# ilirlikalla/Smith-Waterman-FPGA-module

Hardware: AMD Instinct MI355X
Metric: GCUPS (higher is better)
Workload: dtype f16

## Files before the change

smith-waterman-fpga-module_amd/csrc/swbank_bank.h:

```cpp
#ifndef SWBANK_BANK_H
#define SWBANK_BANK_H

#include <dlfcn.h>
#include <hip/hip_runtime.h>
#include <rccl/rccl.h>

#include <algorithm>
#include <cmath>
#include <cstdarg>
#include <cstdio>
#include <cstdlib>
#include <cstring>
#include <atomic>
#include <condition_variable>
#include <functional>
#include <memory>
#include <mutex>
#include <numeric>
#include <thread>
#include <chrono>
#include <vector>
#if defined(__SSE2__)
#include <emmintrin.h>
#endif
#if defined(__x86_64__)
#include <immintrin.h>
#endif

#include "swbank.h"
#include "swbank_align.h"
#include "swbank_internal.h"
#include "swbank_pack.h"

extern "C" int swk_has_variant(int R, int RB, int col0, int prof, int gotoh, int f16);
extern "C" hipError_t swk_launch_wave(int K, int col0, int prof, int gotoh, int f16,
                                      const void* edge_in, void* edge_out, uint32_t ecols,
                                      int accum, const uint8_t* res,
                                      const uint64_t* offs, const uint32_t* lens, size_t n,
                                      const uint32_t* qtab, uint32_t nv, uint32_t S, uint32_t O,
                                      uint32_t E, uint32_t PS, uint32_t pad, int32_t* scores,
                                      int packed, const uint32_t* fb_qtab, uint32_t fb_nv,
                                      uint32_t fb_PS, int32_t fb_thresh,
                                      const SwkWaveSplit* split, uint32_t ulen,
                                      uint32_t ustride, int half, hipStream_t st);
extern "C" hipError_t swk_launch_score(int R, int RB, int col0, int prof, int gotoh, int f16,
                                       const uint8_t* res, const uint64_t* offs,
                                       const uint32_t* lens, size_t n, const uint32_t* qtab,
                                       uint32_t nv, uint32_t S, uint32_t O, uint32_t E,
                                       uint32_t PS, uint32_t pad, int W, int32_t* scores,
                                       const void* edge_in, void* edge_out, uint32_t ecols,
                                       int accum, int packed, const uint32_t* idx,
                                       const uint32_t* nidx, uint32_t idx_base,
                                       const uint32_t* ident, int pair, uint32_t pS1,
                                       uint32_t pS2, uint32_t ulen, uint32_t ustride, uint32_t nq,
                                       uint32_t qwords, size_t sstride, hipStream_t st);
extern "C" unsigned swk_bal_slots(int W, uint32_t PS, int trim);
extern "C" unsigned swk_wave_half_grid(int gotoh, uint32_t prof_bytes, int W);
extern "C" hipError_t swk_bal_plan_uniform(void* plan, uint32_t ntiles, uint32_t K, uint32_t G,
                                           hipStream_t st);
extern "C" hipError_t swk_launch_pair_bal(const uint8_t* res, const uint64_t* offs,
                                          const uint32_t* lens, size_t n, const uint32_t* qtab,
                                          uint32_t nv, uint32_t S, uint32_t O, uint32_t E,
                                          uint32_t PS, uint32_t pad, int W, int32_t* scores,
                                          uint32_t pS1, uint32_t pS2, uint32_t ulen,
                                          uint32_t ustride, uint32_t* flag, uint32_t* state,
                                          uint32_t gen, unsigned grid, const uint32_t* idx,
                                          const uint32_t* nidx, const uint32_t* ident,
                                          const void* plan, uint32_t* fault, uint32_t poll_limit,
                                          uint32_t stall, int trim, uint32_t packed,
                                          const uint32_t* sidx, hipStream_t st);
extern "C" hipError_t swk_best_hit(const int32_t* scores, const uint64_t* ids, size_t n,
                                   unsigned long long* key, uint64_t* out, uint64_t* out_index,
                                   hipStream_t st);
extern "C" hipError_t swk_best_part(const int32_t* scores, size_t n, size_t base,
                                    unsigned long long* key, hipStream_t st);
extern "C" hipError_t swk_best_finalize(const unsigned long long* key, const uint64_t* ids,
                                        uint64_t* out, uint64_t* out_index, hipStream_t st);
extern "C" hipError_t swk_sort_lens(const uint32_t* lens, size_t n, uint32_t max_len,
                                    uint32_t* perm, uint32_t* perm_n, uint32_t* ident,
                                    uint32_t* scratch, hipStream_t st, void* plan = nullptr,
                                    unsigned G = 0);
extern "C" size_t swk_sort_scratch_bytes(void);
extern "C" hipError_t swk_flag_high(const int32_t* scores, size_t n, int32_t thresh,
                                    uint32_t* idx, uint32_t* count, hipStream_t st);
extern "C" size_t swk_i32_waves(size_t n, uint32_t scols, size_t budget_bytes);
extern "C" hipError_t swk_launch_i32(int gotoh, const uint8_t* res, const uint64_t* offs,
                                     const uint32_t* lens, size_t n, int packed,
                                     const uint32_t* idx, const uint32_t* nidx, uint32_t idx_base,
                                     const void* prof, uint32_t nstrips, uint32_t qlen,
                                     uint32_t pad, uint32_t O, uint32_t E, int32_t* scores,
                                     void* scratch, uint32_t scols, size_t waves, hipStream_t st);

extern "C" size_t swk_top_state_words(void);
extern "C" hipError_t swk_top_hits(const int32_t* scores, const uint64_t* ids, size_t n, size_t nq,
                                   size_t k, int32_t min_score, unsigned long long* state,
                                   unsigned long long* keys, uint64_t* hits, int32_t* hit_scores,
                                   uint64_t* hit_ids, uint32_t* counts, hipStream_t st);

inline int env_int(const char* name, int dflt) {
  const char* v = std::getenv(name);
  return (v && *v) ? std::atoi(v) : dflt;
}

struct PhaseTrace {
  const char* path = std::getenv("SWBANK_TRACE_FILE");
  std::chrono::steady_clock::time_point t0 = std::chrono::steady_clock::now();
  std::vector<std::pair<const char*, double>> marks;
  std::mutex mu;
  void mark(const char* what) { mark_at(what, std::chrono::steady_clock::now()); }
  void mark_at(const char* what, std::chrono::steady_clock::time_point t) {
    if (!path) return;
    std::lock_guard<std::mutex> g(mu);
    marks.push_back({what, std::chrono::duration<double, std::micro>(t - t0).count()});
  }
  ~PhaseTrace() {
    if (!path || marks.empty()) return;
    if (FILE* f = std::fopen(path, "a")) {
      for (auto& m : marks) std::fprintf(f, "%s %.1f\n", m.first, m.second);
      std::fprintf(f, "--\n");
      std::fclose(f);
    }
  }
};
inline thread_local PhaseTrace* g_trace = nullptr;
inline void trace_mark(const char* what) {
  if (g_trace) g_trace->mark(what);
}

inline bool poison_buffers() {
  const char* v = std::getenv("SWBANK_POISON");
  return v && v[0] == '1';
}

template <typename T>
struct DevBuf {
  T* p = nullptr;
  size_t cap = 0;
  hipError_t reserve(size_t n) {
    if (n <= cap) return hipSuccess;
    if (p) (void)hipFree(p);
    p = nullptr;
    cap = 0;
    size_t want = std::max<size_t>(n, 64);
    hipError_t e = hipMalloc(reinterpret_cast<void**>(&p), want * sizeof(T));
    if (e == hipSuccess) cap = want;
    if (e == hipSuccess && poison_buffers()) {
      e = hipMemset(p, 0x3C, want * sizeof(T));
      if (e == hipSuccess) e = hipStreamSynchronize(nullptr);
    }
    return e;
  }
  void release() {
    if (p) (void)hipFree(p);
// ... 128 lines not shown
    }
    cv_.notify_one();
  }
  sw_status wait(size_t k) {
    while (done_.load(std::memory_order_acquire) < k) {
#if defined(__SSE2__)
      _mm_pause();
#endif
    }
    return st_.load(std::memory_order_acquire);
  }
  sw_status wait_all() { return wait(posted_); }
  void reset() {
    wait_all();
    posted_ = 0;
    done_.store(0);
    st_.store(SW_OK);
  }

 private:
  void loop(int device) {
    (void)hipSetDevice(device);
    for (;;) {
      std::function<sw_status()> f;
      {
        std::unique_lock<std::mutex> l(m_);
        cv_.wait(l, [&] { return stop_ || !q_.empty(); });
        if (q_.empty()) return;
        f = std::move(q_.front());
        q_.erase(q_.begin());
      }
      if (st_.load(std::memory_order_relaxed) == SW_OK) {
        const sw_status s = f();
        if (s != SW_OK) st_.store(s, std::memory_order_release);
      }
      done_.fetch_add(1, std::memory_order_acq_rel);
    }
  }
  std::mutex m_;
  std::condition_variable cv_;
  std::vector<std::function<sw_status()>> q_;
  bool stop_ = false;
  size_t posted_ = 0;
  std::atomic<size_t> done_{0};
  std::atomic<sw_status> st_{SW_OK};
  std::thread th_;
};

struct sw_bank {
  sw_config cfg{};
  int device = 0;
  int cus = 0;
  hipStream_t stream = nullptr;
  char err[512] = {0};

  bool have_pen = false;
  int alpha = SW_DNA_ALPHA;
  std::vector<int8_t> matrix;
  int32_t gap_open = 0, gap_extend = 0;

  bool have_query = false;
  uint64_t qid = 0;
  std::vector<uint8_t> query;
  std::vector<std::vector<uint8_t>> qset;
  bool mq_ready = false;
  DevBuf<uint32_t> mqtab, mqtab16;
  size_t mq_words = 0;
  DevBuf<uint32_t> mqpair;
  size_t mq_pair_words = 0;
  int mq_pair_segs = 0, mq_pair_rows = 0;
  uint32_t mq_pS1 = 0, mq_pS2 = 0;

  bool dirty = true;
  int R = 32, RB = 4, W = 1, col0 = 0, prof = 0;
  uint32_t S = 0, O = 0, E = 0, nv = 0, PS = 0, pad = 4;
  int32_t smax = 0;
  DevBuf<uint32_t> qtab;
  bool f16 = false;
  uint32_t nv16 = 0, PS16 = 0;
  int32_t f16_neg = 0;
  DevBuf<uint32_t> qtab16;
  DevBuf<uint32_t> qpair;
  uint32_t pair_bytes = 0, pS1 = 0, pS2 = 0;
  DevBuf<uint32_t> fb_idx, fb_cnt;
  bool i32_ready = false;
  uint32_t i32_strips = 0;
  DevBuf<uint2> i32prof, i32scr;
  DevBuf<unsigned long long> best_key;
  bool al_ready = false;
  DevBuf<uint8_t> al_tab, al_res;
  DevBuf<uint2> al_scr;
  DevBuf<uint32_t> al_dirs, al_lens, al_cig, al_list;
  DevBuf<uint64_t> al_offs;
  DevBuf<sw_alignment> al_out;
  DevBuf<SwkAlignPlan> al_plan;
  DevBuf<unsigned long long> top_state, top_keys;
  DevBuf<int32_t> top_scores, top_hsc;
  DevBuf<uint64_t> top_hits;
  DevBuf<uint32_t> top_cnt;
  hipEvent_t ev_top = nullptr;
  struct Seg { int W; size_t off, off16; };
  std::vector<Seg> segs;
  DevBuf<uint2> edge[2];
  int wK = 0;
  int wsegs = 1;
  size_t wseg_words = 0, wseg_words16 = 0;
  uint32_t wPS = 0;
  DevBuf<uint32_t> wtab;
  DevBuf<uint32_t> wtab16;
  uint32_t wPS16 = 0;
  int sK[3] = {0, 0, 0};
  size_t sseg_words[3] = {0, 0, 0}, sseg_words16[3] = {0, 0, 0};
  uint32_t sPS[3] = {0, 0, 0}, sPS16[3] = {0, 0, 0};
  DevBuf<uint32_t> stab[3], stab16[3];
  DevBuf<uint2> sring;
  DevBuf<uint32_t> tprog;

  static constexpr int NSLOT = 3, NDSLOT = 6;
  hipStream_t copy_stream = nullptr;
  hipEvent_t h2d_done[NSLOT] = {}, kern_done[NDSLOT] = {};
  PinBuf hslot[NSLOT], hscores;
  std::vector<std::vector<uint32_t>> mlist;
  std::vector<std::vector<uint8_t>> mstage;
  std::vector<std::vector<uint32_t>> mbad;
  std::vector<hipEvent_t> out_ev;
  hipStream_t out_stream = nullptr;
  hipStream_t stream2 = nullptr;
  hipEvent_t ev_s2 = nullptr;
  double host_pack_ms = 0;
  int feed_dslots = NSLOT;
  DevBuf<uint8_t> dslot[NDSLOT];
  DevBuf<uint32_t> sortscr[NDSLOT];
  DevBuf<uint8_t> sbuf;
  UcBuf sflag;
  DevBuf<SwkStreamChunk> sdrec;
  DevBuf<uint32_t> sctr;
  hipStream_t kstream = nullptr;
  PinBuf srec, shflag{hipHostMallocCoherent};
  PinBuf shscores{hipHostMallocCoherent};
  std::vector<hipEvent_t> sev;
  std::unique_ptr<HostPool> pool;
  std::unique_ptr<Launcher> launcher;

  DevBuf<uint8_t> res;
  DevBuf<uint64_t> offs;
  DevBuf<uint32_t> lens;
  DevBuf<int32_t> scores;
  DevBuf<uint8_t> gres;
  DevBuf<uint64_t> goffs;
  DevBuf<uint32_t> glens;

  char last_kernel[160] = {0};

  int best_kind = 0;
  uint64_t best_id = 0, best_index = 0;
  int32_t best_score = 0;
  DevBuf<uint64_t> best_dev;
  hipEvent_t best_ev = nullptr;

  std::vector<sw_bank*> kids;
  std::unique_ptr<HostPool> dpool;
  std::vector<void*> comms;
  bool rccl_gather = false;
  unsigned pool_threads = 0;
  DevBuf<int32_t> grecv;
  PinBuf hrecv;
// ... 178 lines not shown
```

smith-waterman-fpga-module_amd/csrc/swbank_bank.hip:

```cpp
#include "swbank_bank.h"

sw_status fail(sw_bank* b, sw_status st, const char* fmt, ...) {
  if (b) {
    va_list ap;
    va_start(ap, fmt);
    vsnprintf(b->err, sizeof(b->err), fmt, ap);
    va_end(ap);
  }
  return st;
}

extern "C" int32_t sw_device_count(void) {
  int n = 0;
  if (hipGetDeviceCount(&n) != hipSuccess) return 0;
  return n;
}

static sw_status check_device(int dev) {
  int ndev = 0;
  if (hipGetDeviceCount(&ndev) != hipSuccess || ndev <= 0) return SW_ERR_NO_DEVICE;
  if (dev < 0 || dev >= ndev) return SW_ERR_NO_DEVICE;
  hipDeviceProp_t prop;
  if (hipGetDeviceProperties(&prop, dev) != hipSuccess) return SW_ERR_NO_DEVICE;
  if (std::strncmp(prop.gcnArchName, "gfx950", 6) != 0) return SW_ERR_NO_DEVICE;
// ... 63 lines not shown
        sw_bank_destroy(b);
        return SW_ERR_UNSUPPORTED;
      }
      if (b->comms.empty())
        snprintf(b->err, sizeof(b->err), "RCCL unavailable (%s), gathering with device copies",
                 r.ok ? r.errorString(nr) : r.err);
    }
    (void)hipSetDevice(b->device);
    *out = b;
    return SW_OK;
  }

  int dev = cfg.device;
  if (dev < 0 && hipGetDevice(&dev) != hipSuccess) return SW_ERR_NO_DEVICE;
  const sw_status dst = check_device(dev);
  if (dst != SW_OK) return dst;

  sw_bank* b = new (std::nothrow) sw_bank();
  if (!b) return SW_ERR_NOMEM;
  b->cfg = cfg;
  b->device = dev;
  if (hipSetDevice(dev) != hipSuccess ||
      hipStreamCreateWithFlags(&b->stream, hipStreamNonBlocking) != hipSuccess ||
      hipStreamCreateWithFlags(&b->copy_stream, hipStreamNonBlocking) != hipSuccess ||
      hipStreamCreateWithFlags(&b->out_stream, hipStreamNonBlocking) != hipSuccess ||
      hipStreamCreateWithFlags(&b->stream2, hipStreamNonBlocking) != hipSuccess) {
    for (hipStream_t* x : {&b->stream, &b->copy_stream, &b->out_stream, &b->stream2})
      if (*x) (void)hipStreamDestroy(*x);
    delete b;
    return SW_ERR_HIP;
  }
  b->alpha = cfg.alphabet == SW_ALPHABET_DNA ? SW_DNA_ALPHA : SW_PROTEIN_ALPHA;
  if (hipDeviceGetAttribute(&b->cus, hipDeviceAttributeMultiprocessorCount, dev) != hipSuccess)
    b->cus = 0;
  if (cfg.alphabet == SW_ALPHABET_PROTEIN) {
    int8_t m[SW_PROTEIN_ALPHA * SW_PROTEIN_ALPHA];
    sw_fill_matrix(SW_ALPHABET_PROTEIN, 0, 0, m);
    b->matrix.assign(m, m + sizeof(m));
    b->gap_open = -11;
    b->gap_extend = -1;
    b->have_pen = true;
  }
  *out = b;
  return SW_OK;
}

extern "C" void sw_bank_destroy(sw_bank* b) {
  DevGuard dev_guard(b);
  if (!b) return;
  if (b->is_multi() || !b->comms.empty()) {
    const Rccl& r = rccl();
    for (void* c : b->comms) (void)r.commDestroy(static_cast<ncclComm_t>(c));
    (void)hipSetDevice(b->device);
    if (b->ev_used) (void)hipEventSynchronize(b->ev_used);
    if (b->ev_join) (void)hipEventDestroy(b->ev_join);
    if (b->ev_used) (void)hipEventDestroy(b->ev_used);
    for (sw_bank* k : b->kids) sw_bank_destroy(k);
    b->dpool.reset();
    b->pool.reset();
    (void)hipSetDevice(b->device);
    b->grecv.release();
    b->hrecv.release();
    b->res.release();
    b->offs.release();
    b->lens.release();
    b->dperm.release();
    b->dsort.release();
    delete b;
    return;
  }
  (void)hipSetDevice(b->device);
  if (b->stream) (void)hipStreamSynchronize(b->stream);
  if (b->ev_top) (void)hipEventSynchronize(b->ev_top);
  uint64_t nl;
  double pm, sm;
  (void)sw_bank_timing(b, &nl, &pm, &sm);
  b->faultw.release();
  b->qtab.release();
  b->qtab16.release();
  b->mqtab.release();
  b->mqtab16.release();
  b->mqpair.release();
  b->qpair.release();
  b->stage.release();
  if (b->ev_ready) (void)hipEventDestroy(b->ev_ready);
  if (b->ev_used) (void)hipEventDestroy(b->ev_used);
  if (b->best_ev) (void)hipEventDestroy(b->best_ev);
  if (b->ev_top) (void)hipEventDestroy(b->ev_top);
  if (b->ev_join) (void)hipEventDestroy(b->ev_join);
  for (hipEvent_t e : b->deal_ev) (void)hipEventDestroy(e);
  b->fb_idx.release();
  b->fb_cnt.release();
  b->best_key.release();
  b->best_dev.release();
  b->i32prof.release();
  b->i32scr.release();
  b->al_tab.release();
  b->al_res.release();
  b->al_scr.release();
  b->al_dirs.release();
  b->al_lens.release();
  b->al_cig.release();
  b->al_list.release();
  b->al_offs.release();
  b->al_out.release();
  b->al_plan.release();
  b->top_state.release();
  b->top_keys.release();
  b->top_scores.release();
  b->top_hsc.release();
  b->top_hits.release();
  b->top_cnt.release();
  b->dperm.release();
  b->dsort.release();
  b->bal_state.release();
  b->bal_flag.release();
  b->wbal_state.release();
  b->wbal_flag.release();
  b->bal_plan.release();
  b->wtab.release();
  b->wtab16.release();
  b->tprog.release();
  for (int i = 0; i < 3; ++i) {
    b->stab[i].release();
    b->stab16[i].release();
  }
  b->sring.release();
  b->edge[0].release();
  b->edge[1].release();
  if (b->copy_stream) (void)hipStreamSynchronize(b->copy_stream);
  if (b->out_stream) (void)hipStreamSynchronize(b->out_stream);
  if (b->stream2) (void)hipStreamSynchronize(b->stream2);
  for (hipEvent_t e : b->out_ev) (void)hipEventDestroy(e);
  for (int i = 0; i < sw_bank::NSLOT; ++i) b->hslot[i].release();
  for (int i = 0; i < sw_bank::NDSLOT; ++i) {
    b->dslot[i].release();
    b->sortscr[i].release();
  }
  b->sbuf.release();
  b->sflag.release();
  b->sdrec.release();
  b->sctr.release();
  b->srec.release();
  b->shflag.release();
  b->shscores.release();
  for (hipEvent_t e : b->sev) (void)hipEventDestroy(e);
  for (int i = 0; i < sw_bank::NSLOT; ++i)
    if (b->h2d_done[i]) (void)hipEventDestroy(b->h2d_done[i]);
  for (int i = 0; i < sw_bank::NDSLOT; ++i)
    if (b->kern_done[i]) (void)hipEventDestroy(b->kern_done[i]);
  b->hscores.release();
  b->launcher.reset();
  b->pool.reset();
  if (b->copy_stream) (void)hipStreamDestroy(b->copy_stream);
  if (b->out_stream) (void)hipStreamDestroy(b->out_stream);
  if (b->stream2) (void)hipStreamDestroy(b->stream2);
  if (b->kstream) (void)hipStreamDestroy(b->kstream);
  if (b->ev_s2) (void)hipEventDestroy(b->ev_s2);
  b->res.release();
  b->offs.release();
  b->lens.release();
  b->scores.release();
  b->gres.release();
  b->goffs.release();
  b->glens.release();
  if (b->stream) (void)hipStreamDestroy(b->stream);
// ... 156 lines not shown
  DevGuard dev_guard(b);
  if (!b || !m) return SW_ERR_ARG;
  if (b->is_multi())
    return each_kid(b, [&](sw_bank* k) { return sw_set_matrix(k, m, alpha, gap_open, gap_extend); });
  const int want = b->cfg.alphabet == SW_ALPHABET_DNA ? SW_DNA_ALPHA : SW_PROTEIN_ALPHA;
  if (alpha != want) return fail(b, SW_ERR_ARG, "matrix alphabet %d, bank expects %d", alpha, want);
  return set_matrix_impl(b, m, alpha, gap_open, gap_extend);
}

extern "C" sw_status sw_load_query(sw_bank* b, uint64_t id, const uint8_t* codes, uint32_t len) {
  DevGuard dev_guard(b);
  if (!b || (!codes && len)) return SW_ERR_ARG;
  if (b->is_multi()) {
    const sw_status st = each_kid(b, [&](sw_bank* k) { return sw_load_query(k, id, codes, len); });
    b->qset.clear();
    b->have_query = st == SW_OK;
    return st;
  }
  const uint32_t cap = b->cfg.max_query_len ? b->cfg.max_query_len : SWB_MAX_QUERY;
  if (len > cap)
    return fail(b, SW_ERR_UNSUPPORTED, "query length %u exceeds the bank maximum %u", len, cap);
  for (uint32_t i = 0; i < len; ++i)
    if (codes[i] >= (uint32_t)b->alpha)
      return fail(b, SW_ERR_ARG, "query code %u at %u outside alphabet %d", codes[i], i, b->alpha);
  b->query.assign(codes, codes + len);
  b->qid = id;
  b->qset.clear();
  b->have_query = true;
  b->dirty = true;
  return SW_OK;
}

extern "C" sw_status sw_load_queries(sw_bank* b, size_t nq, const uint64_t* ids,
                                     const uint8_t* codes, const uint64_t* offsets,
                                     const uint32_t* lens) {
  DevGuard dev_guard(b);
  if (!b || nq == 0 || !offsets || !lens) return SW_ERR_ARG;
  if (b->is_multi()) {
    const sw_status st = each_kid(
        b, [&](sw_bank* k) { return sw_load_queries(k, nq, ids, codes, offsets, lens); });
    b->qset = b->kids[0]->qset;
    b->have_query = st == SW_OK;
    return st;
  }
  if (nq > 65536) return fail(b, SW_ERR_UNSUPPORTED, "more than 65536 queries in one set");
  if (nq == 1) return sw_load_query(b, ids ? ids[0] : 0, codes + offsets[0], lens[0]);
  const uint32_t cap = b->cfg.max_query_len ? b->cfg.max_query_len : SWB_MAX_QUERY;
  size_t longest = 0;
  for (size_t i = 0; i < nq; ++i) {
    if (lens[i] > cap)
      return fail(b, SW_ERR_UNSUPPORTED, "query %zu length %u exceeds the bank maximum %u", i,
                  lens[i], cap);
    if (lens[i] && !codes) return fail(b, SW_ERR_ARG, "null query codes");
    for (uint32_t j = 0; j < lens[i]; ++j)
      if (codes[offsets[i] + j] >= (uint32_t)b->alpha)
        return fail(b, SW_ERR_ARG, "query %zu code %u at %u outside alphabet %d", i,
                    codes[offsets[i] + j], j, b->alpha);
    if (lens[i] > lens[longest]) longest = i;
  }
  b->qset.assign(nq, {});
  for (size_t i = 0; i < nq; ++i)
    b->qset[i].assign(codes + offsets[i], codes + offsets[i] + lens[i]);
  b->query = b->qset[longest];
  b->qid = ids ? ids[longest] : 0;
  b->have_query = true;
  b->dirty = true;
  b->mq_ready = false;
  return SW_OK;
}

extern "C" size_t sw_query_count(const sw_bank* b) {
  return !b || !b->have_query ? 0 : b->qset.size() > 1 ? b->qset.size() : 1;
}

static void pair_strides(uint32_t NR, uint32_t& pS1, uint32_t& pS2) {
  const uint32_t B = 4 * NR;
  pS2 = (B + 15) / 16 * 16;
  while ((pS2 / 16) % 16 != 1) pS2 += 16;
  pS1 = (4 * pS2 + B + 15) / 16 * 16;
  while ((pS1 / 16) % 16 != 4) pS1 += 16;
}

static std::vector<uint32_t> pair_table(const uint8_t* q, int qlen, int r0, uint32_t NR,
                                        const int8_t* m, int A, uint32_t pS1, uint32_t pS2) {
  const uint32_t bytes = 16 + 4 * pS1 + 4 * pS2 + 4 * NR;
  std::vector<uint32_t> t(bytes / 4, 0xBC00BC00u);
  auto word = [&](int r, int x, int y) -> uint32_t {
    if (r0 + r >= qlen) return 0xBC00BC00u;
    const int c = q[r0 + r];
    return (uint32_t)f16_score_bits(m[c * A + x]) | (uint32_t)f16_score_bits(m[c * A + y]) << 16;
  };
  for (int x = 0; x < A; ++x)
    for (int y = 0; y < A; ++y) {
      const uint32_t base = (16 + x * pS1 + y * pS2) / 4;
      for (uint32_t k = 0; k + 1 < NR; ++k) t[base + k] = word((int)k + 1, x, y);
    }
  for (int x = 0; x < A; ++x)
    for (int y = 0; y < A; ++y) t[(16 + x * pS1 + y * pS2) / 4 - 1] = word(0, x, y);
  return t;
}

sw_status prepare(sw_bank* b) {
  if (!b->have_pen || !b->have_query)
    return fail(b, SW_ERR_STATE, "load penalties (ld_penalties) and a query (ld_sequence) first");
  if (!b->dirty) return SW_OK;
  const int A = b->alpha;
  const int8_t* m = b->matrix.data();
  int smax = -128, smin = 127;
  for (int i = 0; i < A * A; ++i) {
    smax = std::max<int>(smax, m[i]);
    smin = std::min<int>(smin, m[i]);
  }
  const int S = std::max(0, smax);
  if (S - smin > 254)
    return fail(b, SW_ERR_RANGE, "substitution range [%d, %d] exceeds 254", smin, smax);
  const int o = -b->gap_open, e = -b->gap_extend;
  const bool gotoh = b->cfg.gap_model == SW_GAP_GOTOH;
  if (gotoh && o + e + S > 65535) return fail(b, SW_ERR_RANGE, "gap penalties too large");

  bool lut = A == SW_DNA_ALPHA;
  const int sN = m[4];
  for (int i = 0; lut && i < A; ++i) lut = m[i * A + 4] == sN;
  lut = lut && sN <= 0;
  bool lut_f16 = true;
  for (int i = 0; i < A * A; ++i) {
    const uint16_t bits = f16_score_bits(m[i]);
    lut_f16 = lut_f16 && (bits & 0xFFu) == 0;
  }
  const bool f16_range = -(o + 2 * e + (std::max(0, smax) - smin)) >= -2048;
  const int prof =
      (env_int("SWBANK_PROFILE", 0) || !lut || (!lut_f16 && f16_range)) ? 1 : 0;

  const int qlen = (int)b->query.size();
  const int col0 = (!gotoh && smax > o + e) ? 1 : 0;
  const bool u16_only = gotoh && (!f16_range || env_int("SWBANK_F16", 1) == 0);
  int R = (qlen <= 16 || prof || col0 || u16_only) ? 16 : 32, RB = 4;
  R = env_int("SWBANK_R", R);
  RB = env_int("SWBANK_RB", RB);
  const int max_rows = (R >= 64 ? 8 : 16) * R;
  int seg_rows = qlen > max_rows ? env_int("SWBANK_SEG", max_rows)
                                 : std::max(qlen, 1);
  if (seg_rows % R != 0 && seg_rows < qlen)
    return fail(b, SW_ERR_ARG, "segment rows %d not a multiple of R=%d", seg_rows, R);
  if (!swk_has_variant(R, RB, col0, prof, gotoh ? 1 : 0, 0))
    return fail(b, SW_ERR_UNSUPPORTED, "no kernel variant R=%d RB=%d col0=%d prof=%d gotoh=%d", R,
                RB, col0, prof, (int)gotoh);
  const int Wseg = std::max(1, (seg_rows + R - 1) / R);
  if (Wseg * 64 > (R >= 64 ? 512 : 1024))
    return fail(b, SW_ERR_UNSUPPORTED, "segment of %d rows too tall for one workgroup", seg_rows);

  std::vector<uint32_t> tab;
  std::vector<sw_bank::Seg> segs;
  uint32_t PS = prof ? (uint32_t)((Wseg * R + 15) / 16 * 16) : 0;
  if (prof) PS += (16u + 256u - PS % 256u) % 256u;
  const uint32_t pad = prof ? (uint32_t)A : 4u;
  const uint32_t nv = prof ? 0u : (uint32_t)(uint8_t)(S - sN) * 0x01010101u;
  for (int r0 = 0; r0 < std::max(qlen, 1); r0 += seg_rows) {
    const int rows = std::min(seg_rows, std::max(qlen, 1) - r0);
    const int W = std::max(1, (rows + R - 1) / R);
    segs.push_back({W, tab.size(), 0});
    if (!prof) {
      const size_t base = tab.size();
      tab.resize(base + (size_t)W * R, 0xFFFFFFFFu);
      for (int i = 0; i < rows && r0 + i < qlen; ++i) {
        uint32_t w = 0;
        for (int c = 0; c < 4; ++c)
          w |= (uint32_t)(uint8_t)(S - m[b->query[r0 + i] * A + c]) << (8 * c);
        tab[base + i] = w;
      }
    } else {
      std::vector<uint8_t> qp((size_t)(A + 1) * PS, 0xFF);
      for (int c = 0; c < A; ++c)
        for (int i = 0; i < rows && r0 + i < qlen; ++i)
          qp[(size_t)c * PS + i] = (uint8_t)(S - m[b->query[r0 + i] * A + c]);
      const size_t base = tab.size();
      tab.resize(base + qp.size() / 4);
      std::memcpy(tab.data() + base, qp.data(), qp.size());
    }
  }
  auto f16_hi = [](int v, uint8_t* out) {
    const uint16_t bits = f16_score_bits(v);
    *out = (uint8_t)(bits >> 8);
    return (bits & 0xFFu) == 0 &&
           (int)((float)__builtin_bit_cast(_Float16, bits) * 2048.0f) == v;
  };
  bool f16 = swk_has_variant(R, RB, col0, prof, gotoh ? 1 : 0, 1) != 0;
  std::vector<uint32_t> tab16;
  uint8_t hN = 0;
  uint32_t PS16 = 0;
  if (!prof) {
    f16 = f16 && f16_hi(sN, &hN);
    for (int i = 0; f16 && i < A * A; ++i) {
      uint8_t h;
      f16 = f16_hi(m[i], &h);
    }
  }
  if (f16 && !prof) {
    tab16.assign(tab.size(), 0xBCBCBCBCu);
    for (sw_bank::Seg& sg : segs) {
      const int r0 = (int)(&sg - segs.data()) * seg_rows;
      sg.off16 = sg.off;
      for (int i = 0; i < sg.W * R && r0 + i < qlen && i < seg_rows; ++i) {
        uint32_t w = 0;
        for (int c = 0; c < 4; ++c) {
          uint8_t h;
          f16_hi(m[b->query[r0 + i] * A + c], &h);
          w |= (uint32_t)h << (8 * c);
        }
        tab16[sg.off + i] = w;
      }
    }
  } else if (f16) {
    PS16 = (uint32_t)((2 * Wseg * R + 15) / 16 * 16);
    PS16 += (16u + 256u - PS16 % 256u) % 256u;
    const uint16_t padv = 0xBC00u;
    for (sw_bank::Seg& sg : segs) {
      const int r0 = (int)(&sg - segs.data()) * seg_rows;
      std::vector<uint16_t> qp((size_t)(A + 1) * PS16 / 2, padv);
      for (int c = 0; c < A; ++c)
        for (int i = 0; i < sg.W * R && r0 + i < qlen && i < seg_rows; ++i)
          qp[(size_t)c * PS16 / 2 + i] =
              f16_score_bits(m[b->query[r0 + i] * A + c]);
      sg.off16 = tab16.size();
      tab16.resize(sg.off16 + qp.size() / 2);
      std::memcpy(tab16.data() + sg.off16, qp.data(), qp.size() * 2);
    }
  }
  std::vector<uint32_t> tpair;
  uint32_t pS1 = 0, pS2 = 0, pair_words = 0;
  if (f16 && !prof && !col0 && A == SW_DNA_ALPHA &&
      (gotoh ? R == 16 || R == 32 : R == 32 && segs.size() == 1 && segs[0].W <= 4)) {
    const uint32_t NR = (uint32_t)segs[0].W * R;
    pair_strides(NR, pS1, pS2);
    for (size_t sg = 0; sg < segs.size(); ++sg) {
      const std::vector<uint32_t> t =
          pair_table(b->query.data(), qlen, (int)sg * seg_rows, NR, m, A, pS1, pS2);
      pair_words = (uint32_t)t.size();
      tpair.insert(tpair.end(), t.begin(), t.end());
    }
  }
  const auto wave_tables = [&](int wrows, int nsegs, std::vector<uint32_t>& wt,
                               std::vector<uint32_t>& wt16) {
    for (int sg = 0; sg < nsegs; ++sg) {
      const int r0 = sg * wrows, nr = std::min(wrows, std::max(0, qlen - r0));
      if (!prof) {
        const size_t base = wt.size();
        wt.resize(base + wrows, 0xFFFFFFFFu);
        for (int i = 0; i < nr; ++i) {
          uint32_t w = 0;
          for (int c = 0; c < 4; ++c)
            w |= (uint32_t)(uint8_t)(S - m[b->query[r0 + i] * A + c]) << (8 * c);
          wt[base + i] = w;
        }
        if (f16) {
          const size_t b16 = wt16.size();
          wt16.resize(b16 + wrows, 0xBCBCBCBCu);
          for (int i = 0; i < nr; ++i) {
            uint32_t w = 0;
            for (int c = 0; c < 4; ++c) {
              uint8_t h;
              f16_hi(m[b->query[r0 + i] * A + c], &h);
              w |= (uint32_t)h << (8 * c);
            }
            wt16[b16 + i] = w;
          }
        }
      } else {
        std::vector<uint8_t> qp((size_t)(A + 1) * wrows, 0xFF);
        for (int c = 0; c < A; ++c)
          for (int i = 0; i < nr; ++i)
            qp[(size_t)c * wrows + i] = (uint8_t)(S - m[b->query[r0 + i] * A + c]);
        const size_t base = wt.size();
        wt.resize(base + qp.size() / 4);
        std::memcpy(wt.data() + base, qp.data(), qp.size());
        if (f16) {
          std::vector<uint16_t> q16((size_t)(A + 1) * wrows, 0xBC00u);
          for (int c = 0; c < A; ++c)
            for (int i = 0; i < nr; ++i)
              q16[(size_t)c * wrows + i] = f16_score_bits(m[b->query[r0 + i] * A + c]);
          const size_t b16 = wt16.size();
          wt16.resize(b16 + q16.size() / 2);
          std::memcpy(wt16.data() + b16, q16.data(), q16.size() * 2);
        }
      }
    }
  };
  std::vector<uint32_t> wt, wt16;
  const int wK = qlen <= 256 ? 4 : qlen <= 512 ? 8 : 16;
  const int wrows = 64 * wK;
  const int wsegs = std::max(1, (qlen + wrows - 1) / wrows);
  const uint32_t wPS = prof ? (uint32_t)wrows : 0, wPS16 = prof ? (uint32_t)wrows * 2 : 0;
  wave_tables(wrows, wsegs, wt, wt16);
  std::vector<uint32_t> st[3], st16[3];
  int sK[3] = {0, 0, 0};
  for (int i = 0; i < 3; ++i) {
    sK[i] = (wsegs == 1 && wK >= 8) ? wK / (2 << i) : 0;
    if (sK[i]) wave_tables(64 * sK[i], 2 << i, st[i], st16[i]);
  }
  HIPOK(b, hipSetDevice(b->device));
  if (!b->ev_ready) {
    HIPOK(b, hipEventCreateWithFlags(&b->ev_ready, hipEventDisableTiming));
    HIPOK(b, hipEventCreateWithFlags(&b->ev_used, hipEventDisableTiming));
    HIPOK(b, hipEventRecord(b->ev_ready, b->stream));
    HIPOK(b, hipEventRecord(b->ev_used, b->stream));
  }
  HIPOK(b, hipEventSynchronize(b->ev_ready));
  const size_t nbytes =
      (wt16.size() + wt.size() + st16[0].size() + st[0].size() + st16[1].size() +
       st[1].size() + st16[2].size() + st[2].size() + tab.size() + tab16.size() + tpair.size()) *
      4;
  HIPOK(b, b->stage.reserve(nbytes));
  HIPOK(b, hipStreamWaitEvent(b->stream, b->ev_used, 0));
  size_t at = 0;
  auto upload = [&](DevBuf<uint32_t>& dst, const std::vector<uint32_t>& src) -> hipError_t {
    hipError_t e = dst.reserve(src.size());
    if (e != hipSuccess || src.empty()) return e;
    std::memcpy(b->stage.p + at, src.data(), src.size() * 4);
    e = hipMemcpyAsync(dst.p, b->stage.p + at, src.size() * 4, hipMemcpyHostToDevice, b->stream);
    at += src.size() * 4;
    return e;
  };
  if (!wt16.empty()) HIPOK(b, upload(b->wtab16, wt16));
  HIPOK(b, upload(b->wtab, wt));
  b->wPS16 = wPS16;
  b->wK = wK;
  b->wPS = wPS;
  b->wsegs = wsegs;
  b->wseg_words = wt.size() / wsegs;
  b->wseg_words16 = wt16.empty() ? 0 : wt16.size() / wsegs;
  for (int i = 0; i < 3; ++i) {
    if (!st16[i].empty()) HIPOK(b, upload(b->stab16[i], st16[i]));
    HIPOK(b, upload(b->stab[i], st[i]));
    b->sK[i] = sK[i];
    b->sseg_words[i] = st[i].size() / (2 << i);
    b->sseg_words16[i] = st16[i].size() / (2 << i);
    b->sPS[i] = prof ? (uint32_t)(64 * sK[i]) : 0;
    b->sPS16[i] = prof ? (uint32_t)(128 * sK[i]) : 0;
  }
  HIPOK(b, upload(b->qtab, tab));
  if (f16) HIPOK(b, upload(b->qtab16, tab16));
  if (!tpair.empty()) HIPOK(b, upload(b->qpair, tpair));
  b->pair_bytes = pair_words * 4;
  b->pS1 = pS1;
  b->pS2 = pS2;
  HIPOK(b, hipEventRecord(b->ev_ready, b->stream));
  b->f16 = f16;
  b->nv16 = (uint32_t)hN * 0x01010101u;
  b->PS16 = PS16;
  b->f16_neg = -(o + 2 * e + (S - smin));
  b->R = R;
  b->RB = RB;
  b->W = segs[0].W;
  b->segs = segs;
  b->S = (uint32_t)S;
  b->O = (uint32_t)o;
  b->E = (uint32_t)e;
  b->nv = nv;
  b->PS = PS;
  b->pad = pad;
  b->prof = prof;
  b->smax = smax;
  b->col0 = col0;
  b->i32_ready = false;
  b->al_ready = false;
  b->mq_ready = false;
  b->dirty = false;
  return SW_OK;
}

sw_status prepare_multi(sw_bank* b) {
  if (b->mq_ready) return SW_OK;
  const int A = b->alpha;
  const int8_t* m = b->matrix.data();
  const int R = b->R, S = (int)b->S;
  const size_t words = b->segs.back().off + (size_t)b->segs.back().W * R;
  const int seg_rows = b->segs[0].W * R;
  const size_t nq = b->qset.size();
  std::vector<uint32_t> t16, t8(nq * words, 0xFFFFFFFFu);
  if (b->f16) t16.assign(nq * words, 0xBCBCBCBCu);
  for (size_t i = 0; i < nq; ++i) {
    const std::vector<uint8_t>& qi = b->qset[i];
    for (size_t sg = 0; sg < b->segs.size(); ++sg) {
      const size_t base = i * words + b->segs[sg].off;
      const int r0 = (int)sg * seg_rows;
      for (int j = 0; j < b->segs[sg].W * R && r0 + j < (int)qi.size(); ++j) {
        uint32_t w = 0, h = 0;
        for (int c = 0; c < 4; ++c) {
          const int v = m[qi[r0 + j] * A + c];
          w |= (uint32_t)(uint8_t)(S - v) << (8 * c);
          h |= (uint32_t)(f16_score_bits(v) >> 8) << (8 * c);
        }
        t8[base + j] = w;
        if (b->f16) t16[base + j] = h;
      }
    }
  }
  std::vector<uint32_t> tp;
  b->mq_pair_segs = 0;
  if (b->f16 && !b->prof && !b->gotoh() && !b->col0 && A == SW_DNA_ALPHA &&
      env_int("SWBANK_MQ_PAIR", 1) != 0) {
    const int want = env_int("SWBANK_MQ_PAIR_ROWS", 128);
    const uint32_t NR = want == 128 ? 128 : want == 256 ? 256 : 512;
    b->mq_pair_rows = (int)NR;
    pair_strides(NR, b->mq_pS1, b->mq_pS2);
    const int qmax = (int)b->query.size();
    b->mq_pair_segs = std::max(1, (qmax + (int)NR - 1) / (int)NR);
    for (int sg = 0; sg < b->mq_pair_segs; ++sg)
      for (size_t i = 0; i < nq; ++i) {
        const std::vector<uint32_t> t = pair_table(b->qset[i].data(), (int)b->qset[i].size(),
                                                   sg * (int)NR, NR, m, A, b->mq_pS1, b->mq_pS2);
        b->mq_pair_words = t.size();
        tp.insert(tp.end(), t.begin(), t.end());
      }
  }
  HIPOK(b, hipSetDevice(b->device));
  HIPOK(b, hipEventSynchronize(b->ev_ready));
  HIPOK(b, b->stage.reserve((t8.size() + t16.size() + tp.size()) * 4));
  HIPOK(b, b->mqtab.reserve(t8.size()));
  if (!t16.empty()) HIPOK(b, b->mqtab16.reserve(t16.size()));
  HIPOK(b, hipStreamWaitEvent(b->stream, b->ev_used, 0));
  std::memcpy(b->stage.p, t8.data(), t8.size() * 4);
  HIPOK(b, hipMemcpyAsync(b->mqtab.p, b->stage.p, t8.size() * 4, hipMemcpyHostToDevice,
                          b->stream));
  if (!t16.empty()) {
// ... 133 lines not shown
```

smith-waterman-fpga-module_amd/csrc/swbank_f16_rows.inc:

```
#define SWK_F16M_L_Z0_L0 \
  "v_perm_b32 %[S1], %[nv], %[tb0], %[sel]\n\t" \
  "v_pk_add_f16 %[Db], %[h0], %[S1] clamp\n\t" \
  "v_pk_add_f16 %[DN], %[Da], %[no]\n\t" \
  "v_pk_maximum3_f16 %[h0], %[Da], %[up], %[t0]\n\t" \
  "v_pk_maximum3_f16 %[X], %[DN], %[up], %[t0]\n\t" \
  "v_perm_b32 %[S1], %[nv], %[tb1], %[sel]\n\t" \
  "v_pk_add_f16 %[DN], %[Db], %[no]\n\t" \
  "v_pk_add_f16 %[t0], %[X], %[ne]\n\t" \
  "v_pk_add_f16 %[Da], %[h1], %[S1] clamp\n\t" \
  "v_pk_maximum3_f16 %[h1], %[Db], %[t0], %[t1]\n\t" \
  "v_pk_maximum3_f16 %[X], %[DN], %[t0], %[t1]\n\t" \
  "v_pk_maximum3_f16 %[best], %[best], %[h0], %[h1]\n\t" \
  "v_perm_b32 %[S1], %[nv], %[tb2], %[sel]\n\t" \
  "v_pk_add_f16 %[DN], %[Da], %[no]\n\t" \
  "v_pk_add_f16 %[t1], %[X], %[ne]\n\t" \
  "v_pk_add_f16 %[Db], %[h2], %[S1] clamp\n\t" \
  "v_pk_maximum3_f16 %[h2], %[Da], %[t1], %[t2]\n\t" \
  "v_pk_maximum3_f16 %[X], %[DN], %[t1], %[t2]\n\t" \
  "v_perm_b32 %[S1], %[nv], %[tb3], %[sel]\n\t" \
  "v_pk_add_f16 %[DN], %[Db], %[no]\n\t" \
  "v_pk_add_f16 %[t2], %[X], %[ne]\n\t" \
  "v_pk_add_f16 %[Da], %[h3], %[S1] clamp\n\t" \
  "v_pk_maximum3_f16 %[h3], %[Db], %[t2], %[t3]\n\t" \
  "v_pk_maximum3_f16 %[X], %[DN], %[t2], %[t3]\n\t" \
// ... 1242 lines not shown
  "v_pk_add_f16 %[HN], %[h5], %[noe]\n\t" \
  "v_pk_add_f16 %[FN], %[F], %[ne]\n\t" \
  "v_pk_maximum3_f16 %[t5], 0, %[HN], %[EN]\n\t" \
  "v_pk_maximum3_f16 %[F], 0, %[HN], %[FN]\n\t" \
  "v_pk_maximum3_f16 %[best], %[best], %[h4], %[h5]\n\t" \
  "v_pk_add_f16 %[Db], %[h6], %[p6]\n\t" \
  "v_pk_maximum3_f16 %[h6], %[Da], %[t6], %[F]\n\t" \
  "v_pk_add_f16 %[EN], %[t6], %[ne]\n\t" \
  "v_pk_add_f16 %[HN], %[h6], %[noe]\n\t" \
  "v_pk_add_f16 %[FN], %[F], %[ne]\n\t" \
  "v_pk_maximum3_f16 %[t6], 0, %[HN], %[EN]\n\t" \
  "v_pk_maximum3_f16 %[F], 0, %[HN], %[FN]\n\t" \
  "v_pk_add_f16 %[Da], %[h7], %[p7]\n\t" \
  "v_pk_maximum3_f16 %[h7], %[Db], %[t7], %[F]\n\t" \
  "v_pk_add_f16 %[EN], %[t7], %[ne]\n\t" \
  "v_pk_add_f16 %[HN], %[h7], %[noe]\n\t" \
  "v_pk_add_f16 %[FN], %[F], %[ne]\n\t" \
  "v_pk_maximum3_f16 %[t7], 0, %[HN], %[EN]\n\t" \
  "v_pk_maximum3_f16 %[F], 0, %[HN], %[FN]\n\t" \
  "v_pk_maximum3_f16 %[best], %[best], %[h6], %[h7]\n\t" \
  ""
#define SWK_F16PAIRG_L \
  "v_pk_add_f16 %[Db], %[h0], %[p0]\n\t" \
  "v_pk_maximum3_f16 %[h0], %[Da], %[t0], %[F]\n\t" \
  "v_pk_add_f16 %[EN], %[t0], %[ne]\n\t" \
  "v_pk_add_f16 %[HN], %[h0], %[noe]\n\t" \
  "v_pk_add_f16 %[FN], %[F], %[ne]\n\t" \
  "v_pk_maximum3_f16 %[t0], 0, %[HN], %[EN]\n\t" \
  "v_pk_maximum3_f16 %[F], 0, %[HN], %[FN]\n\t" \
  "v_pk_add_f16 %[Da], %[h1], %[p1]\n\t" \
  "v_pk_maximum3_f16 %[h1], %[Db], %[t1], %[F]\n\t" \
  "v_pk_add_f16 %[EN], %[t1], %[ne]\n\t" \
  "v_pk_add_f16 %[HN], %[h1], %[noe]\n\t" \
  "v_pk_add_f16 %[FN], %[F], %[ne]\n\t" \
  "v_pk_maximum3_f16 %[t1], 0, %[HN], %[EN]\n\t" \
  "v_pk_maximum3_f16 %[F], 0, %[HN], %[FN]\n\t" \
  "v_pk_maximum3_f16 %[best], %[best], %[h0], %[h1]\n\t" \
  "v_pk_add_f16 %[Db], %[h2], %[p2]\n\t" \
  "v_pk_maximum3_f16 %[h2], %[Da], %[t2], %[F]\n\t" \
  "v_pk_add_f16 %[EN], %[t2], %[ne]\n\t" \
  "v_pk_add_f16 %[HN], %[h2], %[noe]\n\t" \
  "v_pk_add_f16 %[FN], %[F], %[ne]\n\t" \
  "v_pk_maximum3_f16 %[t2], 0, %[HN], %[EN]\n\t" \
  "v_pk_maximum3_f16 %[F], 0, %[HN], %[FN]\n\t" \
  "v_pk_add_f16 %[Da], %[h3], %[p3]\n\t" \
  "v_pk_maximum3_f16 %[h3], %[Db], %[t3], %[F]\n\t" \
  "v_pk_add_f16 %[EN], %[t3], %[ne]\n\t" \
  "v_pk_add_f16 %[HN], %[h3], %[noe]\n\t" \
  "v_pk_add_f16 %[FN], %[F], %[ne]\n\t" \
  "v_pk_maximum3_f16 %[t3], 0, %[HN], %[EN]\n\t" \
  "v_pk_maximum3_f16 %[F], 0, %[HN], %[FN]\n\t" \
  "v_pk_maximum3_f16 %[best], %[best], %[h2], %[h3]\n\t" \
  "v_pk_add_f16 %[Db], %[h4], %[p4]\n\t" \
  "v_pk_maximum3_f16 %[h4], %[Da], %[t4], %[F]\n\t" \
  "v_pk_add_f16 %[EN], %[t4], %[ne]\n\t" \
  "v_pk_add_f16 %[HN], %[h4], %[noe]\n\t" \
  "v_pk_add_f16 %[FN], %[F], %[ne]\n\t" \
  "v_pk_maximum3_f16 %[t4], 0, %[HN], %[EN]\n\t" \
  "v_pk_maximum3_f16 %[F], 0, %[HN], %[FN]\n\t" \
  "v_pk_add_f16 %[Da], %[h5], %[p5]\n\t" \
  "v_pk_maximum3_f16 %[h5], %[Db], %[t5], %[F]\n\t" \
  "v_pk_add_f16 %[EN], %[t5], %[ne]\n\t" \
  "v_pk_add_f16 %[HN], %[h5], %[noe]\n\t" \
  "v_pk_add_f16 %[FN], %[F], %[ne]\n\t" \
  "v_pk_maximum3_f16 %[t5], 0, %[HN], %[EN]\n\t" \
  "v_pk_maximum3_f16 %[F], 0, %[HN], %[FN]\n\t" \
  "v_pk_maximum3_f16 %[best], %[best], %[h4], %[h5]\n\t" \
  "v_pk_add_f16 %[Db], %[h6], %[p6]\n\t" \
  "v_pk_maximum3_f16 %[h6], %[Da], %[t6], %[F]\n\t" \
  "v_pk_add_f16 %[EN], %[t6], %[ne]\n\t" \
  "v_pk_add_f16 %[HN], %[h6], %[noe]\n\t" \
  "v_pk_add_f16 %[FN], %[F], %[ne]\n\t" \
  "v_pk_maximum3_f16 %[t6], 0, %[HN], %[EN]\n\t" \
  "v_pk_maximum3_f16 %[F], 0, %[HN], %[FN]\n\t" \
  "s_nop 0\n\t" \
  "v_pk_maximum3_f16 %[h7], %[Db], %[t7], %[F]\n\t" \
  "v_pk_add_f16 %[EN], %[t7], %[ne]\n\t" \
  "v_pk_add_f16 %[HN], %[h7], %[noe]\n\t" \
  "v_pk_add_f16 %[FN], %[F], %[ne]\n\t" \
  "v_pk_maximum3_f16 %[t7], 0, %[HN], %[EN]\n\t" \
  "v_pk_maximum3_f16 %[F], 0, %[HN], %[FN]\n\t" \
  "v_pk_maximum3_f16 %[best], %[best], %[h6], %[h7]\n\t" \
  ""
#define SWK_F16M_F_Z0_L0 \
  "v_pk_fma_f16 %[Db], %[fa0], %[fb0], %[h0] op_sel:[0,1,0] op_sel_hi:[1,0,1] clamp\n\t" \
  "v_pk_add_f16 %[DN], %[Da], %[no]\n\t" \
  "v_pk_maximum3_f16 %[h0], %[Da], %[up], %[t0]\n\t" \
  "v_pk_maximum3_f16 %[X], %[DN], %[up], %[t0]\n\t" \
  "v_pk_add_f16 %[DN], %[Db], %[no]\n\t" \
  "v_pk_add_f16 %[t0], %[X], %[ne]\n\t" \
  "v_pk_fma_f16 %[Da], %[fa1], %[fb1], %[h1] op_sel:[0,1,0] op_sel_hi:[1,0,1] clamp\n\t" \
  "v_pk_maximum3_f16 %[h1], %[Db], %[t0], %[t1]\n\t" \
  "v_pk_maximum3_f16 %[X], %[DN], %[t0], %[t1]\n\t" \
  "v_pk_maximum3_f16 %[best], %[best], %[h0], %[h1]\n\t" \
  "v_pk_add_f16 %[DN], %[Da], %[no]\n\t" \
  "v_pk_add_f16 %[t1], %[X], %[ne]\n\t" \
  "v_pk_fma_f16 %[Db], %[fa2], %[fb2], %[h2] op_sel:[0,1,0] op_sel_hi:[1,0,1] clamp\n\t" \
  "v_pk_maximum3_f16 %[h2], %[Da], %[t1], %[t2]\n\t" \
  "v_pk_maximum3_f16 %[X], %[DN], %[t1], %[t2]\n\t" \
  "v_pk_add_f16 %[DN], %[Db], %[no]\n\t" \
  "v_pk_add_f16 %[t2], %[X], %[ne]\n\t" \
  "v_pk_fma_f16 %[Da], %[fa3], %[fb3], %[h3] op_sel:[0,1,0] op_sel_hi:[1,0,1] clamp\n\t" \
  "v_pk_maximum3_f16 %[h3], %[Db], %[t2], %[t3]\n\t" \
  "v_pk_maximum3_f16 %[X], %[DN], %[t2], %[t3]\n\t" \
  "v_pk_maximum3_f16 %[best], %[best], %[h2], %[h3]\n\t" \
  "v_pk_add_f16 %[DN], %[Da], %[no]\n\t" \
  "v_pk_add_f16 %[t3], %[X], %[ne]\n\t" \
  "v_pk_fma_f16 %[Db], %[fa4], %[fb4], %[h4] op_sel:[0,1,0] op_sel_hi:[1,0,1] clamp\n\t" \
  "v_pk_maximum3_f16 %[h4], %[Da], %[t3], %[t4]\n\t" \
  "v_pk_maximum3_f16 %[X], %[DN], %[t3], %[t4]\n\t" \
  "v_pk_add_f16 %[DN], %[Db], %[no]\n\t" \
  "v_pk_add_f16 %[t4], %[X], %[ne]\n\t" \
  "v_pk_fma_f16 %[Da], %[fa5], %[fb5], %[h5] op_sel:[0,1,0] op_sel_hi:[1,0,1] clamp\n\t" \
  "v_pk_maximum3_f16 %[h5], %[Db], %[t4], %[t5]\n\t" \
  "v_pk_maximum3_f16 %[X], %[DN], %[t4], %[t5]\n\t" \
  "v_pk_maximum3_f16 %[best], %[best], %[h4], %[h5]\n\t" \
  "v_pk_add_f16 %[DN], %[Da], %[no]\n\t" \
  "v_pk_add_f16 %[t5], %[X], %[ne]\n\t" \
  "v_pk_fma_f16 %[Db], %[fa6], %[fb6], %[h6] op_sel:[0,1,0] op_sel_hi:[1,0,1] clamp\n\t" \
  "v_pk_maximum3_f16 %[h6], %[Da], %[t5], %[t6]\n\t" \
  "v_pk_maximum3_f16 %[X], %[DN], %[t5], %[t6]\n\t" \
  "v_pk_add_f16 %[DN], %[Db], %[no]\n\t" \
  "v_pk_add_f16 %[t6], %[X], %[ne]\n\t" \
  "v_pk_fma_f16 %[Da], %[fa7], %[fb7], %[h7] op_sel:[0,1,0] op_sel_hi:[1,0,1] clamp\n\t" \
  "v_pk_maximum3_f16 %[h7], %[Db], %[t6], %[t7]\n\t" \
  "v_pk_maximum3_f16 %[X], %[DN], %[t6], %[t7]\n\t" \
  "v_pk_maximum3_f16 %[best], %[best], %[h6], %[h7]\n\t" \
  "v_pk_add_f16 %[t7], %[X], %[ne]\n\t" \
  ""
#define SWK_F16G_F_L0 \
  "v_pk_fma_f16 %[Db], %[fa0], %[fb0], %[h0] op_sel:[0,1,0] op_sel_hi:[1,0,1]\n\t" \
  "v_pk_maximum3_f16 %[h0], %[Da], %[t0], %[F]\n\t" \
  "v_pk_add_f16 %[EN], %[t0], %[ne]\n\t" \
  "v_pk_add_f16 %[HN], %[h0], %[noe]\n\t" \
  "v_pk_add_f16 %[FN], %[F], %[ne]\n\t" \
  "v_pk_maximum3_f16 %[t0], 0, %[HN], %[EN]\n\t" \
  "v_pk_maximum3_f16 %[F], 0, %[HN], %[FN]\n\t" \
  "v_pk_fma_f16 %[Da], %[fa1], %[fb1], %[h1] op_sel:[0,1,0] op_sel_hi:[1,0,1]\n\t" \
  "v_pk_maximum3_f16 %[h1], %[Db], %[t1], %[F]\n\t" \
  "v_pk_add_f16 %[EN], %[t1], %[ne]\n\t" \
  "v_pk_add_f16 %[HN], %[h1], %[noe]\n\t" \
  "v_pk_add_f16 %[FN], %[F], %[ne]\n\t" \
  "v_pk_maximum3_f16 %[t1], 0, %[HN], %[EN]\n\t" \
  "v_pk_maximum3_f16 %[F], 0, %[HN], %[FN]\n\t" \
  "v_pk_maximum3_f16 %[best], %[best], %[h0], %[h1]\n\t" \
  "v_pk_fma_f16 %[Db], %[fa2], %[fb2], %[h2] op_sel:[0,1,0] op_sel_hi:[1,0,1]\n\t" \
  "v_pk_maximum3_f16 %[h2], %[Da], %[t2], %[F]\n\t" \
  "v_pk_add_f16 %[EN], %[t2], %[ne]\n\t" \
  "v_pk_add_f16 %[HN], %[h2], %[noe]\n\t" \
  "v_pk_add_f16 %[FN], %[F], %[ne]\n\t" \
  "v_pk_maximum3_f16 %[t2], 0, %[HN], %[EN]\n\t" \
  "v_pk_maximum3_f16 %[F], 0, %[HN], %[FN]\n\t" \
  "v_pk_fma_f16 %[Da], %[fa3], %[fb3], %[h3] op_sel:[0,1,0] op_sel_hi:[1,0,1]\n\t" \
  "v_pk_maximum3_f16 %[h3], %[Db], %[t3], %[F]\n\t" \
  "v_pk_add_f16 %[EN], %[t3], %[ne]\n\t" \
  "v_pk_add_f16 %[HN], %[h3], %[noe]\n\t" \
  "v_pk_add_f16 %[FN], %[F], %[ne]\n\t" \
  "v_pk_maximum3_f16 %[t3], 0, %[HN], %[EN]\n\t" \
  "v_pk_maximum3_f16 %[F], 0, %[HN], %[FN]\n\t" \
  "v_pk_maximum3_f16 %[best], %[best], %[h2], %[h3]\n\t" \
  "v_pk_fma_f16 %[Db], %[fa4], %[fb4], %[h4] op_sel:[0,1,0] op_sel_hi:[1,0,1]\n\t" \
  "v_pk_maximum3_f16 %[h4], %[Da], %[t4], %[F]\n\t" \
  "v_pk_add_f16 %[EN], %[t4], %[ne]\n\t" \
  "v_pk_add_f16 %[HN], %[h4], %[noe]\n\t" \
  "v_pk_add_f16 %[FN], %[F], %[ne]\n\t" \
  "v_pk_maximum3_f16 %[t4], 0, %[HN], %[EN]\n\t" \
// ... 322 lines not shown
```

smith-waterman-fpga-module_amd/csrc/swbank_kcommon.h:

```cpp
#ifndef SWBANK_KCOMMON_H
#define SWBANK_KCOMMON_H
#include <hip/hip_runtime.h>
#include <stdint.h>

#include <algorithm>
#include <cstdlib>
#include <mutex>
#include <type_traits>
#include <vector>

#include "swbank_internal.h"

#ifndef SWK_TAIL_TOP
#define SWK_TAIL_TOP 1
#endif
#ifndef SWK_PRIO_ROT
#define SWK_PRIO_ROT 1
#endif
#ifndef SWK_PRIO_SHIFT
#define SWK_PRIO_SHIFT 18
#endif

#ifndef SWK_PRIO_END
#define SWK_PRIO_END 3
// ... 498 lines not shown
  const uint32_t la = lens[a], lb = lens[b];
  t.llo = va ? la : 0u;
  t.lhi = vb ? lb : 0u;
  if constexpr (MIX) {
    if (packed == SWK_PACK_MIXED) {
      const uint32_t* o32 = reinterpret_cast<const uint32_t*>(offs);
      t.plo = la ? mixed_ptr(res, o32[a]) : reinterpret_cast<const uint8_t*>(lens);
      t.phi = lb ? mixed_ptr(res, o32[b]) : reinterpret_cast<const uint8_t*>(lens);
      return t;
    }
  }
  t.plo = la ? res + offs[a] : reinterpret_cast<const uint8_t*>(lens);
  t.phi = lb ? res + offs[b] : reinterpret_cast<const uint8_t*>(lens);
  return t;
}

template <int C = 8>
__device__ __forceinline__ void tile_chunks(const Lane2& t, size_t tlo, size_t thi, size_t n,
                                            int& nch, int& nfull, int& ncl) {
  uint32_t Lmax = max(t.llo, t.lhi);
  uint32_t Lmin = min(tlo < n ? t.llo : ~0u, thi < n ? t.lhi : ~0u);
#pragma unroll
  for (int off = 32; off >= 1; off >>= 1) {
    Lmax = max(Lmax, (uint32_t)__shfl_xor((int)Lmax, off));
    Lmin = min(Lmin, (uint32_t)__shfl_xor((int)Lmin, off));
  }
  const int lx = (int)__builtin_amdgcn_readfirstlane(Lmax);
  nch = max(1, (lx + C - 1) / C);
  ncl = lx == 0 ? C : lx - C * (nch - 1);
  const uint32_t lm = __builtin_amdgcn_readfirstlane(Lmin);
  nfull = lm == ~0u ? 0 : (int)(lm / C);
}

struct ScoreArgs {
  const uint8_t* res;
  const uint64_t* offs;
  const uint32_t* lens;
  size_t n;
  const uint32_t* qtab;
  uint32_t nv;
  uint32_t S, O, E;
  uint32_t PS;
  uint32_t pad;
  int32_t* scores;
  const uint2* edge_in;
  uint2* edge_out;
  uint32_t ecols;
  uint32_t accum;
  uint32_t packed;
  const uint32_t* idx;
  const uint32_t* nidx;
  uint32_t idx_base;
  const uint32_t* ident;
  uint32_t pS1, pS2;
  uint32_t f16_noe, f16_ne, f16_no;
  const uint32_t* fb_qtab;
  uint32_t fb_nv, fb_PS;
  int32_t fb_thresh;
  uint32_t split_blocks;
  uint32_t split_P;
  uint32_t main_pairs;
  const uint32_t* split_qtab;
  const uint32_t* split_fb_qtab;
  uint32_t split_words, split_fb_words, split_PS, split_fb_PS;
  uint2* split_ring;
  uint32_t ulen, ustride;
  uint32_t nq, qwords;
  size_t sstride;
  const SwkStreamChunk* sc;
  const uint32_t* hflag;
  uint32_t* dflag;
  uint32_t* tctr;
  uint32_t nsc;
  uint32_t* bal_flag;
  uint32_t* bal_state;
  const uint4* bal_plan;
  uint32_t bal_gen;
  uint32_t* tail_prog;
  uint32_t tail_pairs, tail_cols;
  uint32_t* fault;
  uint32_t poll_limit, stall;
  uint32_t wbal_blocks, wbal_grid;
  const uint32_t* sidx;
};
static_assert(sizeof(ScoreArgs) == 376, "ScoreArgs layout (kernel argument block) changed");

__device__ __forceinline__ void report_fault(uint32_t* fault, uint32_t bit) {
  if (fault) __hip_atomic_store(fault + __builtin_ctz(bit), bit, __ATOMIC_RELAXED,
                                __HIP_MEMORY_SCOPE_SYSTEM);
}

typedef __attribute__((address_space(3))) void* lds_void_ptr;
typedef __attribute__((address_space(1))) void* glob_void_ptr;

#define SWK_RING_ROW 65

template <int C = 8>
__device__ __forceinline__ void dma_edge_chunk(const uint2* src, uint2* dst, int lane) {
  const uint32_t* s = reinterpret_cast<const uint32_t*>(src) + lane;
#pragma unroll
  for (int q = 0; q < 2 * C; ++q)
    __builtin_amdgcn_global_load_lds(
        (glob_void_ptr)(s + q * 64),
        (lds_void_ptr)(reinterpret_cast<uint32_t*>(dst + (q >> 1) * SWK_RING_ROW) + (q & 1) * 64),
        4, 0, 0);
}

template <int C = 8>
__device__ __forceinline__ int tile_nch(const uint8_t* res, const uint32_t* lens, size_t n,
                                        int tile, int lane, uint32_t packed, const uint32_t* idx,
                                        uint32_t ulen, uint32_t ustride) {
  const size_t a = (size_t)tile * SWB_TILE + lane, b = a + 64;
  auto len = [&](size_t k) -> uint32_t {
    if (k >= n) return 0u;
    if (ustride) return ulen;
    if (idx) k = idx[k];
    return packed == SWK_PACK_RECORDS ? record_len(res + k * SWB_RECORD) : lens[k];
  };
  uint32_t L = max(len(a), len(b));
#pragma unroll
  for (int off = 32; off >= 1; off >>= 1) L = max(L, (uint32_t)__shfl_xor((int)L, off));
  return max(1, (int)((__builtin_amdgcn_readfirstlane(L) + C - 1) / C));
}

#ifndef SWK_STREAM_POLL
#define SWK_STREAM_POLL 64
#endif
#ifndef SWK_STREAM_POLL_ALL
#define SWK_STREAM_POLL_ALL 0
#endif
__device__ __forceinline__ uint32_t stream_mode(const uint32_t* hflag, uint32_t* dflag, int c,
                                                int nsc, int lane) {
  for (int it = 0; it < (1 << 20); ++it) {
    uint32_t v = __builtin_amdgcn_readfirstlane(
        __hip_atomic_load(dflag + c, __ATOMIC_ACQUIRE, __HIP_MEMORY_SCOPE_AGENT));
    if (v) {
      __builtin_amdgcn_fence(__ATOMIC_ACQUIRE, "");
      return v;
    }
    if ((SWK_STREAM_POLL_ALL || threadIdx.x < 64) &&
        (it == 0 || ((it + (int)blockIdx.x) % SWK_STREAM_POLL) == 0)) {
      v = __builtin_amdgcn_readfirstlane(
          __hip_atomic_load(hflag + c, __ATOMIC_ACQUIRE, __HIP_MEMORY_SCOPE_SYSTEM));
      if (v) {
        if (lane == 0) __hip_atomic_store(dflag + c, v, __ATOMIC_RELEASE, __HIP_MEMORY_SCOPE_AGENT);
        return v;
      }
    }
    __builtin_amdgcn_s_sleep(16);
  }
  if (lane == 0) {
    __hip_atomic_store(dflag + c, SWK_STREAM_ABORT, __ATOMIC_RELAXED, __HIP_MEMORY_SCOPE_AGENT);
    __hip_atomic_store(const_cast<uint32_t*>(hflag) + nsc + c, SWK_STREAM_ABORT,
                       __ATOMIC_RELAXED, __HIP_MEMORY_SCOPE_SYSTEM);
  }
  return SWK_STREAM_ABORT;
}


inline int cached_occupancy(const void* fn, int threads, size_t lds, int dev, int* cus) {
  struct Entry { const void* fn; int threads; size_t lds; int dev, occ, cus; };
  static std::mutex m;
  static std::vector<Entry> cache;
  std::lock_guard<std::mutex> g(m);
  for (const Entry& e : cache)
    if (e.fn == fn && e.threads == threads && e.lds == lds && e.dev == dev) {
      *cus = e.cus;
      return e.occ;
// ... 23 lines not shown
```

smith-waterman-fpga-module_amd/csrc/swbank_ktile.hip:

```cpp
#include "swbank_kcommon.h"

namespace swk {

#ifndef SWK_TRIM_BREAK
#define SWK_TRIM_BREAK 1
#endif
template <int R, int RB, bool COL0, bool PROF, bool GOTOH, bool F16, bool PAIR = false,
          bool MQ = false, bool STREAM = false, int C = 8, bool BAL = false, bool TRIM = false>
__global__ void __launch_bounds__(R >= 64 ? 512 : 1024) score_kernel(const ScoreArgs a) {
  static_assert(!BAL || (!MQ && !STREAM && !COL0), "balanced ranges: one query, resident batch");
  static_assert(!TRIM || (BAL && PAIR), "trimmed last chunks: the balanced pair kernel");
  static_assert(!MQ || !PROF, "several queries: row-LUT or pair-table variants");
  static_assert(!STREAM || (!MQ && !PROF), "streamed batches: single-query LUT / pair variants");
  static_assert(C == 8 || (C == 4 && PAIR && !STREAM), "4-column chunks: pair tables only");
  static_assert(!PAIR || ((R == 32 || (R == 16 && GOTOH)) && F16 && !PROF && !COL0 &&
                          (!GOTOH || !MQ)),
                "PAIR: f16, merged R = 32 or Gotoh R = 16 / 32 (one query)");
  extern __shared__ __attribute__((aligned(16))) uint32_t smem[];
  const int lane = threadIdx.x & 63;
  const int wave = __builtin_amdgcn_readfirstlane(threadIdx.x >> 6);
  const int W = __builtin_amdgcn_readfirstlane(blockDim.x >> 6);
  const bool seg_in = a.edge_in != nullptr, seg_out = a.edge_out != nullptr;
  uint32_t* bestsh = smem + (PAIR ? a.PS / 4 : 0);
  constexpr int RS = SWK_RING_ROW;
  uint2* ein = reinterpret_cast<uint2*>(bestsh + W * SWB_TILE);
  uint2* ring = ein + (seg_in ? 2 * C * RS : 0);
  uint8_t* prof = reinterpret_cast<uint8_t*>(ring + (size_t)(W > 1 ? 2 * (W - 1) : 1) * C * RS);

  size_t n = a.n;
  const uint32_t* idx = a.idx;
  if (idx && a.ident && __builtin_amdgcn_readfirstlane(*a.ident)) idx = nullptr;
  const uint32_t* sidx = TRIM ? a.sidx : nullptr;
  if (TRIM && sidx && a.ident && __builtin_amdgcn_readfirstlane(*a.ident)) sidx = nullptr;
  if (idx) {
    const uint32_t cnt = __builtin_amdgcn_readfirstlane(*a.nidx);
    n = cnt > a.idx_base ? min(a.n, (size_t)(cnt - a.idx_base)) : 0;
  }
  const int ntiles = (int)((n + SWB_TILE - 1) / SWB_TILE);
  const int G = (int)gridDim.x;
  const int nunits = MQ ? ntiles * (int)a.nq : ntiles;
  int total = 0;
  uint32_t packed = a.packed;
  int* sq = reinterpret_cast<int*>(prof);
  int bs = 0, bo = 0, be = 0, bf = 0;
  if constexpr (BAL) {
    const uint4 p0 = a.bal_plan[blockIdx.x], p1 = a.bal_plan[blockIdx.x + 1];
    bs = (int)__builtin_amdgcn_readfirstlane(p0.x), bo = (int)__builtin_amdgcn_readfirstlane(p0.y);
    be = (int)__builtin_amdgcn_readfirstlane(p1.x), bf = (int)__builtin_amdgcn_readfirstlane(p1.y);
    total = (int)__builtin_amdgcn_readfirstlane(p1.z - p0.z);
  }
  const auto bal_visit = [&](int v, int& t, int& c0, int& c1) {
    const int bK = -1;
    const int bfirst = bo ? bs + 1 : bs;
    const int hh = bf > 0 ? 1 : 0;
    if (v < hh) {
      t = be, c0 = 0, c1 = bf;
    } else if (v - hh < be - bfirst) {
      t = bfirst + v - hh, c0 = 0, c1 = bK;
    } else if (v - hh == be - bfirst && bo > 0) {
      t = bs, c0 = bo, c1 = bK;
    } else {
      t = nunits, c0 = 0, c1 = 1;
    }
    t = __builtin_amdgcn_readfirstlane(t);
    c0 = __builtin_amdgcn_readfirstlane(c0);
    c1 = __builtin_amdgcn_readfirstlane(c1);
  };
  if constexpr (BAL) {
  } else if constexpr (STREAM) {
    total = (int)blockIdx.x < ntiles ? (1 << 30) : 0;
  } else {
    for (int u = blockIdx.x; u < nunits; u += G)
      total += tile_nch<C>(a.res, a.lens, n, !MQ ? u : PAIR ? u / (int)a.nq : u % ntiles, lane,
                        packed, idx, a.ulen, a.ustride);
  }
  const SwkStreamChunk* const ssc = a.sc;
  const int snc = (int)a.nsc;
  int scur = -1, st0 = 0;
  uint32_t scn = 0, sro_lo = 0, sro_hi = 0, smode = SWK_PACK_STREAM;
  const uint32_t* cperm = nullptr;
  const uint32_t* wperm = nullptr;
  int wst0 = 0;
  const auto stream_tile = [&](int t, uint32_t& pk) -> Lane2 {
    if (t >= ntiles) {
      pk = SWK_PACK_STREAM;
      Lane2 e;
      e.llo = e.lhi = 0u;
      e.plo = e.phi = a.res;
      return e;
    }
    int c = scur < 0 ? 0 : scur;
    while (c + 1 < snc && t >= (int)ssc[c + 1].tile0) ++c;
    if (c != scur) {
      scur = __builtin_amdgcn_readfirstlane(c);
      st0 = __builtin_amdgcn_readfirstlane((int)ssc[c].tile0);
      scn = __builtin_amdgcn_readfirstlane(
          (uint32_t)((c + 1 < snc ? (size_t)ssc[c + 1].tile0 * SWB_TILE : n) -
                     (size_t)st0 * SWB_TILE));
      sro_lo = __builtin_amdgcn_readfirstlane(ssc[c].res_off_lo);
      sro_hi = __builtin_amdgcn_readfirstlane(ssc[c].res_off_hi);
      const uint32_t md = stream_mode(a.hflag, a.dflag, c, snc, lane);
      smode = a.ulen == 0 ? SWK_PACK_MIXED
                          : md == SWK_PACK_NIBBLE ? SWK_PACK_NIBBLE : SWK_PACK_STREAM;
      if (md == SWK_STREAM_ABORT && a.ulen == 0) {
        const uint64_t z = (uint64_t)__builtin_amdgcn_readfirstlane(ssc[c].zero_off256) * 256u;
        sro_lo = (uint32_t)z;
        sro_hi = (uint32_t)(z >> 32);
      }
    }
    pk = smode;
    const uint8_t* base = a.res + ((size_t)sro_hi << 32 | sro_lo);
    if (a.ulen == 0) {
      const uint32_t* co = reinterpret_cast<const uint32_t*>(base);
      const uint32_t* cl = co + scn;
      cperm = cl + scn;
      return lane_targets<true>(base + (((size_t)scn * 12 + 15) & ~(size_t)15),
                                reinterpret_cast<const uint64_t*>(co), cl, scn, t - st0, lane, pk,
                                cperm, 0u, 0u);
    }
    return lane_targets<true>(base, nullptr, nullptr, scn, t - st0, lane, pk, nullptr, a.ulen,
                               pk == SWK_PACK_NIBBLE ? (a.ulen + 1) / 2 : (a.ulen + 3) / 4);
  };

  int unit = blockIdx.x, q = 0;
  int tile = unit;
  int vc0 = 0, vend = 0;
  if constexpr (BAL) {
    bal_visit(0, tile, vc0, vend);
    unit = tile;
  }
  if constexpr (MQ) {
    if (unit < nunits) {
      q = PAIR ? unit % (int)a.nq : unit / ntiles;
      tile = PAIR ? unit / (int)a.nq : unit - q * ntiles;
    }
  }
  Lane2 cur;
  if constexpr (STREAM) {
    cur = stream_tile(tile, packed);
    wperm = cperm;
    wst0 = st0;
  } else {
    cur = lane_targets<!MQ>(a.res, a.offs, a.lens, n, tile, lane, packed, idx, a.ulen,
                            a.ustride);
  }
  int nch, nfull, ncl;
  tile_chunks<C>(cur, (size_t)tile * SWB_TILE + lane, (size_t)tile * SWB_TILE + lane + 64, n, nch,
              nfull, ncl);
  (void)ncl;
  if constexpr (BAL) {
    if (vend >= 0 && vend < nch) ncl = C;
    nch = vend < 0 ? nch : vend;
  }
  const uint32_t S = a.S;

  for (int i = threadIdx.x; i < W * SWB_TILE; i += blockDim.x) bestsh[i] = 0;
  const f16x2 NOE2 = as_f16x2(as_u16x2(a.f16_noe)), NE2 = as_f16x2(as_u16x2(a.f16_ne)),
              NO2 = as_f16x2(as_u16x2(a.f16_no));
  if (wave == 0) {
    if (lane < C)
      ring[lane * RS + 64] = F16 ? make_uint2(0u, GOTOH ? 0u : as_u32(as_u16x2(NOE2)))
                                 : make_uint2(S | (S << 16), 0u);
    if (seg_in)
      dma_edge_chunk<C>(a.edge_in + (size_t)(MQ ? unit : tile) * a.ecols * 64, ein, lane);
  }
  uint32_t nv = a.nv;
  uint32_t tab[PROF || PAIR ? 1 : R];
  if constexpr (PAIR) {
    const uint4* src = reinterpret_cast<const uint4*>(a.qtab + (MQ ? (size_t)q * a.qwords : 0));
    for (uint32_t i = threadIdx.x; i < a.PS / 16; i += blockDim.x)
      reinterpret_cast<uint4*>(smem)[i] = src[i];
  } else if constexpr (PROF) {
    const uint32_t words = (a.pad + 1) * a.PS / 16;
    const uint4* src = reinterpret_cast<const uint4*>(a.qtab);
    for (uint32_t i = threadIdx.x; i < words; i += blockDim.x)
      reinterpret_cast<uint4*>(prof)[i] = src[i];
  } else {
    asm volatile("" : "+v"(nv));
#pragma unroll
    for (int r = 0; r < R; ++r)
      tab[r] = __builtin_amdgcn_readfirstlane(a.qtab[(MQ ? (size_t)q * a.qwords : 0) + wave * R + r]);
  }
  const u16x2 S2 = {(unsigned short)S, (unsigned short)S};
  const u16x2 O2 = {(unsigned short)a.O, (unsigned short)a.O};
  const u16x2 E2 = {(unsigned short)a.E, (unsigned short)a.E};
  const uint32_t oes = a.O + a.E + S;
  const u16x2 OES2 = {(unsigned short)oes, (unsigned short)oes};
  const u16x2 H0 = F16 ? (u16x2){0, 0} : S2;
  const u16x2 X0 = (F16 && !GOTOH) ? as_u16x2(NOE2) : (u16x2){0, 0};

  u16x2 Hl[R], Xl[R];
#pragma unroll
  for (int r = 0; r < R; ++r) {
    Hl[r] = H0;
    Xl[r] = X0;
  }
  u16x2 best = {0, 0};
  u16x2 prevUpH = H0;
  uint2 rlo, rhi;
  load_raw<C, !MQ>(cur, vc0, vc0 < nfull, a.pad, packed, rlo, rhi);
  if (STREAM && threadIdx.x == 0) sq[W] = total;
  __syncthreads();

  typedef unsigned int u32x4 __attribute__((ext_vector_type(4)));
  typedef __attribute__((address_space(3))) const u32x4 lds_u4;
  typedef __attribute__((address_space(3))) const uint32_t lds_u32;
  const auto ld4 = [](uint32_t addr) { return __builtin_bit_cast(uint4, *(lds_u4*)(size_t)addr); };
  const auto ld1 = [](uint32_t addr) {
    return __atomic_load_n((lds_u32*)(size_t)addr, __ATOMIC_RELAXED);
  };
  const uint32_t wofs = (uint32_t)wave * R * 4 + (uint32_t)(size_t)(lds_void_ptr)smem;
  const u16x2 pS12 = {(unsigned short)a.pS1, (unsigned short)a.pS2};
  const auto pair_addr = [&](uint32_t wl, uint32_t wh, int sh) {
    const uint32_t sel = (uint32_t)(sh >> 3) | 0x0C00u | ((uint32_t)(4 + (sh >> 3)) << 16) |
                         0x0C000000u;
    const u16x2 ab = __builtin_elementwise_min(as_u16x2(__builtin_amdgcn_perm(wh, wl, sel)),
                                               (u16x2){4, 4});
    return __builtin_amdgcn_udot2(ab, pS12, wofs, false);
  };
  uint32_t acur = 0, pw = 0;
  uint4 pA0 = {0, 0, 0, 0}, pA1 = {0, 0, 0, 0};
  if constexpr (PAIR) {
    acur = pair_addr(rlo.x, rhi.x, 0);
    pA0 = ld4(acur + 16);
    pA1 = ld4(acur + 32);
    pw = ld1(acur + 12);
  }
  (void)pA0; (void)pA1; (void)pw; (void)acur; (void)wofs;

  const uint32_t pbase = (uint32_t)wave * R;
  const uint32_t padc = a.pad;
  int bal_pend = 0;
  const auto bal_store = [&](int g_to) {
    uint32_t ol = (uint32_t)lane;
    asm volatile("" : "+v"(ol));
    uint32_t* sp = a.bal_state + ((size_t)g_to * W + wave) * (2 * R + 2) * 64 + ol;
#pragma unroll
    for (int r = 0; r < R; ++r) {
      __hip_atomic_store(sp + r * 64, as_u32(Hl[r]), __ATOMIC_RELAXED, __HIP_MEMORY_SCOPE_AGENT);
      __hip_atomic_store(sp + (R + r) * 64, as_u32(Xl[r]), __ATOMIC_RELAXED,
                         __HIP_MEMORY_SCOPE_AGENT);
    }
    __hip_atomic_store(sp + 2 * R * 64, as_u32(prevUpH), __ATOMIC_RELAXED, __HIP_MEMORY_SCOPE_AGENT);
    __hip_atomic_store(sp + (2 * R + 1) * 64, as_u32(best), __ATOMIC_RELAXED,
                       __HIP_MEMORY_SCOPE_AGENT);
    bal_pend = 2;
  };
  const auto bal_flag_out = [&]() {
    asm volatile("s_waitcnt vmcnt(0)" ::: "memory");
    if (lane == 0 && blockIdx.x + 1 != a.stall)
      __hip_atomic_store(a.bal_flag + ((size_t)blockIdx.x + 1) * W + wave, a.bal_gen,
                         __ATOMIC_RELAXED, __HIP_MEMORY_SCOPE_AGENT);
  };
#if SWK_STAMPS
  uint64_t st_bload = 0;
#endif
  const auto bal_load = [&]() {
#if SWK_STAMPS
    const uint64_t sb0 = __builtin_amdgcn_s_memtime();
#endif
    const uint32_t* fl = a.bal_flag + (size_t)blockIdx.x * W + wave;
    uint32_t it = 0;
    for (; it < a.poll_limit; ++it) {
      if (__builtin_amdgcn_readfirstlane(
              __hip_atomic_load(fl, __ATOMIC_RELAXED, __HIP_MEMORY_SCOPE_AGENT)) == a.bal_gen)
        break;
      __builtin_amdgcn_s_sleep(8);
    }
    if (it == a.poll_limit && lane == 0) report_fault(a.fault, SWK_FAULT_BAL);
    asm volatile("s_waitcnt vmcnt(0)" ::: "memory");
    uint32_t ol = (uint32_t)lane;
    asm volatile("" : "+v"(ol));
    const uint32_t* sp = a.bal_state + ((size_t)blockIdx.x * W + wave) * (2 * R + 2) * 64 + ol;
#pragma unroll
    for (int r = 0; r < R; ++r) {
      Hl[r] = as_u16x2(__hip_atomic_load(sp + r * 64, __ATOMIC_RELAXED, __HIP_MEMORY_SCOPE_AGENT));
      Xl[r] = as_u16x2(
          __hip_atomic_load(sp + (R + r) * 64, __ATOMIC_RELAXED, __HIP_MEMORY_SCOPE_AGENT));
    }
    prevUpH = as_u16x2(
        __hip_atomic_load(sp + 2 * R * 64, __ATOMIC_RELAXED, __HIP_MEMORY_SCOPE_AGENT));
// ... 9 lines not shown
  int nch_n = 1, nfull_n = 0, ncl_n = C;
  uint32_t packed_n = packed;
#if SWK_PRIO_ROT
  const uint32_t prq = (uint32_t)((blockIdx.x * 4ull) / gridDim.x);
  uint32_t prio = 4;
#endif
#if SWK_STAMPS
  uint64_t st_t0 = __builtin_amdgcn_s_memtime(), st_act = 0, st_idle = 0, st_bar = 0;
  uint64_t st_p = st_t0;
#endif
  for (int ph = 0;; ++ph) {
    if constexpr (STREAM) total = __builtin_amdgcn_readfirstlane(sq[W]);
    if (ph >= total + W - 1) break;
#if SWK_PRIO_ROT
    if (W <= 8)
      prio_rotate(prq, prio,
                  SWK_PRIO_END && ph >= total - (total >> SWK_PRIO_END_FRAC)
                      ? SWK_PRIO_SHIFT - SWK_PRIO_END : SWK_PRIO_SHIFT);

#endif
    const int g = ph - wave;
    if (g >= 0 && g < total) {
      const uint2 clo = rlo, chi = rhi;
      const bool last = c + 1 == nch;
      int nunit = (MQ ? unit : tile) + G;
      int nc0 = 0, nvend = 0;
      if constexpr (BAL) {
        if (last) bal_visit(k + 1, nunit, nc0, nvend);
      }
      if constexpr (STREAM) {
        if (last) {
          if (wave == 0) {
            int nt = 0;
            if (lane == 0) nt = G + (int)atomicAdd(a.tctr, 1u);
            nt = min(__builtin_amdgcn_readfirstlane(nt), ntiles);
            if (lane == 0) {
              sq[(k + 1) % W] = nt;
              if (nt >= ntiles) sq[W] = g + 1;
            }
            nunit = nt;
          } else {
            nunit = __builtin_amdgcn_readfirstlane(sq[(k + 1) % W]);
          }
        }
      }
      int ntile = nunit, nqq = q;
      if constexpr (MQ) {
        if (nunit < nunits) {
          if constexpr (PAIR) {
            ntile = nunit / (int)a.nq;
          } else {
            ntile = tile + G;
            while (ntile >= ntiles) {
              ntile -= ntiles;
              ++nqq;
            }
          }
        }
      }
      if (!last) {
        load_raw<C, !MQ>(cur, c + 1, c + 1 < nfull, a.pad, packed, rlo, rhi);
      } else if (nunit < nunits) {
        if constexpr (STREAM) cur = stream_tile(ntile, packed_n);
        else
          cur = lane_targets<!MQ>(a.res, a.offs, a.lens, n, ntile, lane, packed, idx, a.ulen,
                                  a.ustride);
        tile_chunks<C>(cur, (size_t)ntile * SWB_TILE + lane, (size_t)ntile * SWB_TILE + lane + 64,
                    n, nch_n, nfull_n, ncl_n);
        if (BAL && nvend >= 0 && nvend < nch_n) ncl_n = C;
        if (BAL && nvend < 0) nvend = nch_n;
        load_raw<C, !MQ>(cur, nc0, nc0 < nfull_n, a.pad, STREAM ? packed_n : packed, rlo, rhi);
      }
      const int slot = g & 1;
      if (seg_in && wave == 0 && (last ? nunit < nunits : (MQ ? unit : tile) < nunits))
        dma_edge_chunk<C>(a.edge_in + ((size_t)(last ? nunit : MQ ? unit : tile) * a.ecols +
                                    (size_t)(last ? 0 : c + 1) * C) * 64,
                       ein + (size_t)((g + 1) & 1) * C * RS, lane);
      uint2* rin = wave > 0 ? ring + ((size_t)((wave - 1) * 2 + slot) * C) * RS + lane
                   : seg_in ? ein + (size_t)slot * C * RS + lane
                            : ring + 64;
      uint2* rout = wave < W - 1 ? ring + ((size_t)(wave * 2 + slot) * C) * RS + lane
                    : W > 1      ? rin
                                 : ring + lane;
      uint2 rv = rin[0];
      ProfLookup16<PROF && F16 ? R : 2> lkq;
      (void)lkq;
      const int ncols = TRIM && c + 1 == nch ? ncl : C;
      bool trimmed = false;
      (void)ncols;
#pragma unroll
      for (int jj = 0; jj < C; ++jj) {
        if (TRIM && jj > 0 && __builtin_expect(jj >= ncols, 0)) {
          trimmed = true;
#if SWK_TRIM_BREAK
          break;
#else
          continue;
#endif
        }
        const u16x2 upH = as_u16x2(rv.x);
        u16x2 upX = as_u16x2(rv.y);
        if (jj + 1 < C) rv = rin[(jj + 1) * RS];
        u16x2 diag = prevUpH;
        prevUpH = upH;
        const uint32_t wlo = jj < 4 ? clo.x : clo.y, whi = jj < 4 ? chi.x : chi.y;
        if constexpr (PROF && F16) {
          const auto load16 = [&](int j, ProfLookup16<R>& out) {
            const uint32_t wl = j < 4 ? clo.x : clo.y, wh = j < 4 ? chi.x : chi.y;
            const uint32_t blo = min((wl >> (8 * (j & 3))) & 0xFFu, padc);
            const uint32_t bhi = min((wh >> (8 * (j & 3))) & 0xFFu, padc);
            const uint4* plo = reinterpret_cast<const uint4*>(prof + __umul24(blo, a.PS) + 2 * pbase);
            const uint4* phi = reinterpret_cast<const uint4*>(prof + __umul24(bhi, a.PS) + 2 * pbase);
#pragma unroll
            for (int q = 0; q < R / 8; ++q) {
              const uint4 x = plo[q], y = phi[q];
              out.lo[4 * q] = x.x; out.lo[4 * q + 1] = x.y; out.lo[4 * q + 2] = x.z;
              out.lo[4 * q + 3] = x.w;
              out.hi[4 * q] = y.x; out.hi[4 * q + 1] = y.y; out.hi[4 * q + 2] = y.z;
              out.hi[4 * q + 3] = y.w;
            }
          };
          ProfLookup16<R> lk;
          if (jj == 0) load16(0, lk);
          else lk = lkq;
          if (jj + 1 < C) load16(jj + 1, lkq);
          __builtin_amdgcn_sched_barrier(0);
          if (COL0 && jj == 0 && c == 0)
            column_f16<R, RB, GOTOH, true>(lk, diag, upX, Hl, Xl, best, NOE2, NE2, NO2);
          else
            column_f16<R, RB, GOTOH, false>(lk, diag, upX, Hl, Xl, best, NOE2, NE2, NO2);
        } else if constexpr (PROF) {
          ProfLookup<R> lk;
          const uint32_t blo = min((wlo >> (8 * (jj & 3))) & 0xFFu, padc);
          const uint32_t bhi = min((whi >> (8 * (jj & 3))) & 0xFFu, padc);
          const uint4* plo = reinterpret_cast<const uint4*>(prof + __umul24(blo, a.PS) + pbase);
          const uint4* phi = reinterpret_cast<const uint4*>(prof + __umul24(bhi, a.PS) + pbase);
#pragma unroll
          for (int q = 0; q < R / 16; ++q) {
            const uint4 x = plo[q], y = phi[q];
            lk.lo[4 * q] = x.x; lk.lo[4 * q + 1] = x.y; lk.lo[4 * q + 2] = x.z;
            lk.lo[4 * q + 3] = x.w;
            lk.hi[4 * q] = y.x; lk.hi[4 * q + 1] = y.y; lk.hi[4 * q + 2] = y.z;
            lk.hi[4 * q + 3] = y.w;
          }
          __builtin_amdgcn_sched_barrier(0);
          if constexpr (GOTOH) {
            u16x2 uH = upH;
            column_gotoh<R, RB>(lk, diag, uH, upX, Hl, Xl, best, S2, OES2, E2);
          } else if (COL0 && jj == 0 && c == 0) {
            column_merged<R, RB, true>(lk, diag, upX, Hl, Xl, best, S2, O2, E2);
          } else {
            column_merged<R, RB, false>(lk, diag, upX, Hl, Xl, best, S2, O2, E2);
          }
        } else if constexpr (PAIR) {
          const uint32_t nwl = jj + 1 < C ? (jj + 1 < 4 ? clo.x : clo.y) : rlo.x;
          const uint32_t nwh = jj + 1 < C ? (jj + 1 < 4 ? chi.x : chi.y) : rhi.x;
          const int nsh = jj + 1 < C ? 8 * ((jj + 1) & 3) : 0;
          uint32_t Da, Db, X, DN, IN;
          const uint32_t noe = as_u32(as_u16x2(NOE2)), ne = as_u32(as_u16x2(NE2)),
                 no = as_u32(as_u16x2(NO2));
          u16x2 bst = best;
          u16x2 F = upX;
#define SWK_PAIR_HT(B)                                                                        \
  [h0] "+v"(Hl[B]), [h1] "+v"(Hl[B + 1]), [h2] "+v"(Hl[B + 2]), [h3] "+v"(Hl[B + 3]),          \
      [h4] "+v"(Hl[B + 4]), [h5] "+v"(Hl[B + 5]), [h6] "+v"(Hl[B + 6]), [h7] "+v"(Hl[B + 7]),  \
      [t0] "+v"(Xl[B]), [t1] "+v"(Xl[B + 1]), [t2] "+v"(Xl[B + 2]), [t3] "+v"(Xl[B + 3]),      \
      [t4] "+v"(Xl[B + 4]), [t5] "+v"(Xl[B + 5]), [t6] "+v"(Xl[B + 6]), [t7] "+v"(Xl[B + 7]),  \
      [Db] "=&v"(Db), [best] "+v"(bst)
#define SWK_PAIR_OUT(B, DA) SWK_PAIR_HT(B), [Da] DA(Da), [X] "=&v"(X), [DN] "=&v"(DN), [IN] "=&v"(IN)
#define SWK_PAIR_OUTG(B, DA)                                                                  \
  SWK_PAIR_HT(B), [Da] DA(Da), [EN] "=&v"(X), [HN] "=&v"(DN), [FN] "=&v"(IN), [F] "+v"(F)
#define SWK_PAIR_IN(P0, P1)                                                                   \
  [p0] "v"(P0.x), [p1] "v"(P0.y), [p2] "v"(P0.z), [p3] "v"(P0.w), [p4] "v"(P1.x),             \
      [p5] "v"(P1.y), [p6] "v"(P1.z), [p7] "v"(P1.w), [noe] "s"(noe), [ne] "s"(ne), [no] "s"(no)
#define SWK_PAIR_BLOCK(KIND, B, P0, P1)                                                       \
  if constexpr (GOTOH) {                                                                      \
    if constexpr (KIND == 0)                                                                  \
      asm volatile(SWK_F16PAIRG_F : SWK_PAIR_OUTG(B, "=&v")                                   \
                   : SWK_PAIR_IN(P0, P1), [dg] "v"(diag), [pw] "v"(pw));                   \
    else if constexpr (KIND == 1)                                                             \
      asm volatile(SWK_F16PAIRG_M : SWK_PAIR_OUTG(B, "+v") : SWK_PAIR_IN(P0, P1));         \
    else                                                                                      \
      asm volatile(SWK_F16PAIRG_L : SWK_PAIR_OUTG(B, "+v") : SWK_PAIR_IN(P0, P1));         \
  } else {                                                                                    \
    if constexpr (KIND == 0)                                                                  \
      asm volatile(SWK_F16PAIR_F : SWK_PAIR_OUT(B, "=&v")                                     \
                   : SWK_PAIR_IN(P0, P1), [up] "v"(upX), [dg] "v"(diag), [pw] "v"(pw));                 \
    else if constexpr (KIND == 1)                                                             \
      asm volatile(SWK_F16PAIR_M : SWK_PAIR_OUT(B, "+v") : SWK_PAIR_IN(P0, P1), [up] "v"(Xl[B - 1]));   \
    else                                                                                      \
      asm volatile(SWK_F16PAIR_L : SWK_PAIR_OUT(B, "+v") : SWK_PAIR_IN(P0, P1), [up] "v"(Xl[B - 1]));   \
  }
          uint4 pB0 = ld4(acur + 48), pB1 = ld4(acur + 64);
          __builtin_amdgcn_sched_barrier(0);
          SWK_PAIR_BLOCK(0, 0, pA0, pA1)
          if constexpr (R == 32) {
            pA0 = ld4(acur + 80);
            pA1 = ld4(acur + 96);
            __builtin_amdgcn_sched_barrier(0);
            SWK_PAIR_BLOCK(1, 8, pB0, pB1)
            pB0 = ld4(acur + 112);
            pB1 = ld4(acur + 128);
            __builtin_amdgcn_sched_barrier(0);
            SWK_PAIR_BLOCK(1, 16, pA0, pA1)
          }
          acur = pair_addr(nwl, nwh, nsh);
          pA0 = ld4(acur + 16);
          pA1 = ld4(acur + 32);
          pw = ld1(acur + 12);
          __builtin_amdgcn_sched_barrier(0);
          SWK_PAIR_BLOCK(2, R - 8, pB0, pB1)
#undef SWK_PAIR_BLOCK
#undef SWK_PAIR_HT
#undef SWK_PAIR_OUT
#undef SWK_PAIR_OUTG
#undef SWK_PAIR_IN
          (void)Db; (void)X; (void)DN; (void)IN;
          best = bst;
          upX = GOTOH ? F : Xl[R - 1];
        } else if constexpr (F16) {
          const uint32_t sel16 = 0x0Cu | ((uint32_t)(jj & 3) << 8) | (0x0Cu << 16) |
                                 ((uint32_t)(4 + (jj & 3)) << 24);
          const LutLookup<R> lk{tab, nv, __builtin_amdgcn_perm(whi, wlo, sel16) | 0x000C000Cu};
          __builtin_amdgcn_sched_barrier(0);
          if (COL0 && jj == 0 && c == 0)
            column_f16<R, RB, GOTOH, true>(lk, diag, upX, Hl, Xl, best, NOE2, NE2, NO2);
          else
            column_f16<R, RB, GOTOH, false>(lk, diag, upX, Hl, Xl, best, NOE2, NE2, NO2);
        } else {
          const uint32_t sel =
              (uint32_t)(jj & 3) | ((uint32_t)(4 + (jj & 3)) << 16) | 0x0C000C00u;
          const LutLookup<R> lk{tab, nv, __builtin_amdgcn_perm(whi, wlo, sel) | 0x0C000C00u};
          __builtin_amdgcn_sched_barrier(0);
          if constexpr (GOTOH) {
            u16x2 uH = upH;
            column_gotoh<R, RB>(lk, diag, uH, upX, Hl, Xl, best, S2, OES2, E2);
          } else if (COL0 && jj == 0 && c == 0) {
            column_merged<R, RB, true>(lk, diag, upX, Hl, Xl, best, S2, O2, E2);
          } else {
            column_merged<R, RB, false>(lk, diag, upX, Hl, Xl, best, S2, O2, E2);
          }
        }
        asm volatile("" : "+v"(best));
        rout[jj * RS] = make_uint2(as_u32(Hl[R - 1]), as_u32(upX));
      }
      if constexpr (PAIR && TRIM) {
        if (trimmed) {
          acur = pair_addr(rlo.x, rhi.x, 0);
          pA0 = ld4(acur + 16);
          pA1 = ld4(acur + 32);
          pw = ld1(acur + 12);
        }
      }
      (void)trimmed;
      if (seg_out && wave == W - 1) {
        uint2* dst = a.edge_out + ((size_t)(MQ ? unit : tile) * a.ecols + (size_t)c * C) * 64 + lane;
#pragma unroll
        for (int jj = 0; jj < C; ++jj) dst[jj * 64] = rout[jj * RS];
      }
      if (last) {
        if (BAL && k == 0 && bf > 0) {
          bal_store((int)blockIdx.x + 1);
        } else {
        uint32_t* bs = bestsh + (k % W) * SWB_TILE;
        atomicMax(&bs[lane], (uint32_t)best.x);
        atomicMax(&bs[lane + 64], (uint32_t)best.y);
        if (wave == W - 1) {
          const size_t tlo = (size_t)tile * SWB_TILE + lane, thi = tlo + 64;
          int32_t blo = (int32_t)bs[lane], bhi = (int32_t)bs[lane + 64];
          bs[lane] = 0;
          bs[lane + 64] = 0;
          if constexpr (F16) {
            blo = f16_unscore((uint32_t)blo);
            bhi = f16_unscore((uint32_t)bhi);
          }
          const uint32_t* sx = TRIM && sidx ? sidx : idx;
          size_t slo = sx && tlo < n ? sx[tlo] : tlo;
          size_t shi = sx && thi < n ? sx[thi] : thi;
          if constexpr (STREAM) {
            if (wperm) {
              const size_t b0 = (size_t)wst0 * SWB_TILE;
              if (tlo < n) slo = b0 + wperm[tlo - b0];
              if (thi < n) shi = b0 + wperm[thi - b0];
            }
          }
          int32_t* qsc = MQ ? a.scores + (size_t)q * a.sstride : a.scores;
          if (a.accum) {
            if (tlo < n) blo = max(blo, qsc[slo]);
            if (thi < n) bhi = max(bhi, qsc[shi]);
          }
          if (tlo < n) qsc[slo] = blo;
          if (thi < n) qsc[shi] = bhi;
        }
        }
#pragma unroll
        for (int r = 0; r < R; ++r) {
          Hl[r] = H0;
          Xl[r] = X0;
        }
        best = (u16x2){0, 0};
        prevUpH = H0;
        tile = ntile;
        if constexpr (STREAM) {
          packed = packed_n;
          wperm = cperm;
          wst0 = st0;
        }
        if constexpr (MQ && PAIR) unit = nunit;
        if constexpr (MQ && !PAIR) {
          unit = nunit;
          if (nqq != q) {
            q = nqq;
#pragma unroll
            for (int r = 0; r < R; ++r)
              tab[r] = __builtin_amdgcn_readfirstlane(a.qtab[(size_t)q * a.qwords + wave * R + r]);
          }
        }
        nch = nch_n;
        nfull = nfull_n;
        ncl = ncl_n;
        c = 0;
        if constexpr (BAL) {
          c = nc0;
          nch = nvend;
          if (nc0 > 0) bal_load();
        }
        ++k;
      } else {
        ++c;
      }
    }
    if constexpr (BAL) {
      if (bal_pend > 0 && --bal_pend == 0) bal_flag_out();
    }
#if SWK_STAMPS
    const bool st_own = g >= 0 && g < total;
    const uint64_t st_b = __builtin_amdgcn_s_memtime();
    (st_own ? st_act : st_idle) += st_b - st_p;
#endif
    __syncthreads();
#if SWK_STAMPS
    st_p = __builtin_amdgcn_s_memtime();
    (st_own ? st_bar : st_idle) += st_p - st_b;
#endif
  }
  if constexpr (BAL) {
    if (bal_pend > 0) bal_flag_out();
  }
#if SWK_STAMPS
  uint64_t* const g_stamps = STREAM ? nullptr : reinterpret_cast<uint64_t*>(a.tctr);
  if (lane == 0 && g_stamps) {
    uint64_t* o = g_stamps + ((size_t)blockIdx.x * 16 + wave) * 16;
    unsigned hw = 0;
    asm volatile("s_getreg_b32 %0, hwreg(HW_REG_HW_ID)" : "=s"(hw));
    o[0] = st_t0;
    o[1] = __builtin_amdgcn_s_memtime();
    o[2] = st_act;
    o[3] = st_idle;
    o[4] = st_bar;
    o[5] = hw;
    unsigned xcc = 0;
    asm volatile("s_getreg_b32 %0, hwreg(HW_REG_XCC_ID)" : "=s"(xcc));
    o[6] = (uint64_t)total;
    o[7] = (uint64_t)(xcc & 15);
    o[8] = st_bload;
  }
#endif
}

static size_t tile_ring_entries(int W, int C, bool seg_in) {
  return (size_t)((W > 1 ? 2 * (W - 1) : 1) + (seg_in ? 2 : 0)) * C * SWK_RING_ROW;
}

template <int R, int RB, bool COL0, bool PROF, bool GOTOH, bool F16, bool PAIR = false,
          bool MQ = false, bool STREAM = false, int C = 8, bool BAL = false, bool TRIM = false>
static hipError_t launch_score(const ScoreArgs& a, int W, uint32_t prof_bytes, hipStream_t st,
                               unsigned bal_grid = 0) {
  const size_t ntiles = (a.n + SWB_TILE - 1) / SWB_TILE * (MQ ? a.nq : 1);
  const size_t lds = (size_t)W * SWB_TILE * 4 + tile_ring_entries(W, C, a.edge_in != nullptr) * 8 +
                     (PROF ? prof_bytes : 0) + (PAIR ? a.PS : 0) + (STREAM ? 256 : 0);
  auto fn = &score_kernel<R, RB, COL0, PROF, GOTOH, F16, PAIR, MQ, STREAM, C, BAL, TRIM>;
  static bool attr_set = false;
  if (!attr_set) {
    hipError_t e = hipFuncSetAttribute(reinterpret_cast<const void*>(fn),
                                       hipFuncAttributeMaxDynamicSharedMemorySize, 160 * 1024);
    if (e != hipSuccess) return e;
    attr_set = true;
  }
  if (lds > 160 * 1024) return hipErrorInvalidConfiguration;
  unsigned grid = BAL ? bal_grid
                      : persistent_grid(reinterpret_cast<const void*>(fn), ntiles, 64 * W, lds);
#if SWK_STAMPS
  if (!STREAM && g_stamps_host) {
    ScoreArgs b = a;
    b.tctr = reinterpret_cast<uint32_t*>(g_stamps_host);
    hipLaunchKernelGGL(fn, dim3(grid), dim3(64 * W), (unsigned)lds, st, b);
    return hipGetLastError();
  }
#endif
  if (MQ && PAIR) grid = std::max(a.nq, grid / a.nq * a.nq);
  if (BAL && (grid == 0 || ntiles < 2 * (size_t)grid)) return hipErrorInvalidConfiguration;
  hipLaunchKernelGGL(fn, dim3(grid), dim3(64 * W), (unsigned)lds, st, a);
  return hipGetLastError();
}

}

#define SWK_VARIANTS(X)                                                                       \
  X(16, 4, 0, 0, 0, 0) X(16, 4, 1, 0, 0, 0) X(32, 4, 0, 0, 0, 0) X(32, 4, 1, 0, 0, 0)         \
  X(32, 8, 0, 0, 0, 0) X(64, 4, 0, 0, 0, 0) X(64, 4, 1, 0, 0, 0)                              \
  X(16, 4, 0, 0, 1, 0) X(32, 4, 0, 0, 1, 0) X(64, 4, 0, 0, 1, 0)                              \
  X(16, 4, 0, 1, 0, 0) X(16, 4, 1, 1, 0, 0) X(32, 4, 0, 1, 0, 0) X(32, 4, 1, 1, 0, 0)         \
  X(64, 4, 0, 1, 0, 0) X(64, 4, 1, 1, 0, 0)                                                   \
  X(16, 4, 0, 1, 1, 0) X(32, 4, 0, 1, 1, 0) X(64, 4, 0, 1, 1, 0)                              \
  X(16, 4, 0, 0, 0, 1) X(16, 4, 1, 0, 0, 1) X(32, 4, 0, 0, 0, 1) X(64, 4, 0, 0, 0, 1)         \
  X(16, 4, 0, 0, 1, 1)                                                                        \
  X(16, 4, 0, 1, 0, 1) X(16, 4, 1, 1, 0, 1) X(16, 4, 0, 1, 1, 1) X(32, 4, 0, 0, 1, 1)


extern "C" int swk_has_variant(int R, int RB, int col0, int prof, int gotoh, int f16) {
#define SWK_HAS(RR, BB, C0, PF, GT, FH) \
  if (R == RR && RB == BB && col0 == C0 && prof == PF && gotoh == GT && f16 == FH) return 1;
  SWK_VARIANTS(SWK_HAS)
#undef SWK_HAS
  return 0;
}

extern "C" hipError_t swk_launch_score(int R, int RB, int col0, int prof, int gotoh, int f16,
                                       const uint8_t* res, const uint64_t* offs,
                                       const uint32_t* lens, size_t n, const uint32_t* qtab,
                                       uint32_t nv, uint32_t S, uint32_t O, uint32_t E,
                                       uint32_t PS, uint32_t pad, int W, int32_t* scores,
                                       const void* edge_in, void* edge_out, uint32_t ecols,
                                       int accum, int packed, const uint32_t* idx,
                                       const uint32_t* nidx, uint32_t idx_base,
                                       const uint32_t* ident, int pair, uint32_t pS1,
                                       uint32_t pS2, uint32_t ulen, uint32_t ustride,
                                       uint32_t nq, uint32_t qwords, size_t sstride,
                                       hipStream_t st) {
  if (n == 0) return hipSuccess;
  swk::ScoreArgs a{res,  offs, lens, n,  qtab, nv, S,
                   O,    E,    PS,   pad, scores, static_cast<const uint2*>(edge_in),
                   static_cast<uint2*>(edge_out), ecols, (uint32_t)accum, (uint32_t)packed,
                   idx, nidx, idx_base, ident, pS1, pS2,
                   swk::f16_pair(-(int)(O + E)), swk::f16_pair(-(int)E),
                   swk::f16_pair(-(int)O), nullptr, 0u, 0u, 0};
  a.ulen = ulen;
  a.ustride = ustride;
  a.nq = nq;
  a.qwords = qwords;
  a.sstride = sstride;
  const uint32_t prof_bytes = (pad + 1) * PS;
  if (nq > 1 && pair) {
    if (R == 32 && f16 && !prof && !gotoh && !col0 && (W > 4 || a.edge_in || a.edge_out))
      return swk::launch_score<32, 4, false, false, false, true, true, true, false, 4>(a, W, 0, st);
    if (R == 32 && f16 && !prof && !gotoh && !col0)
      return swk::launch_score<32, 4, false, false, false, true, true, true>(a, W, 0, st);
    return hipErrorInvalidValue;
  }
  if (nq > 1) {
#define SWK_MQ_CASE(RR, GT, FH)                                                                  \
  if (R == RR && RB == 4 && !col0 && !prof && !pair && gotoh == GT && f16 == FH)                 \
    return swk::launch_score<RR, 4, false, false, (GT != 0), (FH != 0), false, true>(a, W, 0, st);
    SWK_MQ_CASE(32, 0, 1) SWK_MQ_CASE(32, 0, 0) SWK_MQ_CASE(16, 0, 1) SWK_MQ_CASE(16, 0, 0)
    SWK_MQ_CASE(16, 1, 1) SWK_MQ_CASE(16, 1, 0) SWK_MQ_CASE(32, 1, 1) SWK_MQ_CASE(32, 1, 0)
#undef SWK_MQ_CASE
    return hipErrorInvalidValue;
  }
  if (pair) {
    if (R == 32 && f16 && !prof && !gotoh && !col0)
      return swk::launch_score<32, 4, false, false, false, true, true>(a, W, 0, st);
#define SWK_GPAIR(RR)                                                                         \
    if (R == RR && f16 && !prof && gotoh && !col0) {                                          \
      const hipError_t e = a.edge_in || a.edge_out                                            \
          ? hipErrorInvalidConfiguration                                                      \
          : swk::launch_score<RR, 4, false, false, true, true, true>(a, W, 0, st);            \
      if (e != hipErrorInvalidConfiguration) return e;                                        \
      return swk::launch_score<RR, 4, false, false, true, true, true, false, false, 4>(a, W, 0, \
                                                                                         st); \
    }
    SWK_GPAIR(32) SWK_GPAIR(16)
#undef SWK_GPAIR
    return hipErrorInvalidValue;
  }
#define SWK_CASE(RR, BB, C0, PF, GT, FH)                                                      \
  if (R == RR && RB == BB && col0 == C0 && prof == PF && gotoh == GT && f16 == FH)            \
    return swk::launch_score<RR, BB, (C0 != 0), (PF != 0), (GT != 0), (FH != 0)>(a, W,        \
                                                                               prof_bytes, st);
  SWK_VARIANTS(SWK_CASE)
#undef SWK_CASE
  return hipErrorInvalidValue;
}

#if SWK_STAMPS
extern "C" void swk_set_stamps(void* p) { swk::g_stamps_host = static_cast<uint64_t*>(p); }
#endif

namespace swk {
__global__ void __launch_bounds__(256) bal_plan_uniform(uint4* plan, uint32_t ntiles, uint32_t K,
                                                        uint32_t G) {
  for (uint32_t g = threadIdx.x; g <= G; g += blockDim.x) {
    const uint64_t A = (uint64_t)ntiles * K * g / G;
    plan[g] = make_uint4((uint32_t)(A / K), (uint32_t)(A % K), (uint32_t)A, 0u);
  }
}
}

extern "C" hipError_t swk_bal_plan_uniform(void* plan, uint32_t ntiles, uint32_t K, uint32_t G,
                                           hipStream_t st) {
  if (!plan || K == 0 || G == 0 || (uint64_t)ntiles * K >= (1ull << 31)) return hipErrorInvalidValue;
  hipLaunchKernelGGL(swk::bal_plan_uniform, dim3(1), dim3(256), 0, st, static_cast<uint4*>(plan),
                     ntiles, K, G);
  return hipGetLastError();
}

extern "C" unsigned swk_bal_slots(int W, uint32_t PS, int trim) {
  const void* fn =
      trim ? reinterpret_cast<const void*>(
                 &swk::score_kernel<32, 4, false, false, false, true, true, false, false, 8, true,
                                    true>)
           : reinterpret_cast<const void*>(
                 &swk::score_kernel<32, 4, false, false, false, true, true, false, false, 8, true>);
  if (hipFuncSetAttribute(fn, hipFuncAttributeMaxDynamicSharedMemorySize, 160 * 1024) !=
      hipSuccess)
    return 0;
  const size_t lds = (size_t)W * SWB_TILE * 4 + swk::tile_ring_entries(W, 8, false) * 8 + PS;
  int dev = 0, cus = 0;
  if (hipGetDevice(&dev) != hipSuccess) return 0;
  const int occ = swk::cached_occupancy(fn, 64 * W, lds, dev, &cus);
  return occ > 0 && cus > 0 ? (unsigned)(occ * cus) : 0u;
}

extern "C" hipError_t swk_launch_pair_bal(const uint8_t* res, const uint64_t* offs,
                                          const uint32_t* lens, size_t n, const uint32_t* qtab,
                                          uint32_t nv, uint32_t S, uint32_t O, uint32_t E,
                                          uint32_t PS, uint32_t pad, int W, int32_t* scores,
                                          uint32_t pS1, uint32_t pS2, uint32_t ulen,
                                          uint32_t ustride, uint32_t* flag, uint32_t* state,
                                          uint32_t gen, unsigned grid, const uint32_t* idx,
                                          const uint32_t* nidx, const uint32_t* ident,
                                          const void* plan, uint32_t* fault, uint32_t poll_limit,
                                          uint32_t stall, int trim, uint32_t packed,
                                          const uint32_t* sidx, hipStream_t st) {
  if (n == 0) return hipSuccess;
  if (W > 4 || !flag || !state || !plan || !fault || poll_limit == 0 || (idx && !nidx) ||
      (packed != SWK_PACK_BYTES && packed != SWK_PACK_NIBBLE) || (sidx && (!trim || idx)))
    return hipErrorInvalidValue;
  swk::ScoreArgs a{res,  offs, lens, n,  qtab, nv, S,
                   O,    E,    PS,   pad, scores, nullptr, nullptr, 0u, 0u, packed,
                   idx, nidx, 0u, ident, pS1, pS2,
                   swk::f16_pair(-(int)(O + E)), swk::f16_pair(-(int)E),
                   swk::f16_pair(-(int)O), nullptr, 0u, 0u, 0};
  a.ulen = ulen;
  a.ustride = ustride;
  a.nq = 1;
  a.bal_flag = flag;
  a.bal_state = state;
  a.bal_gen = gen;
  a.bal_plan = static_cast<const uint4*>(plan);
  a.fault = fault;
  a.poll_limit = poll_limit;
  a.stall = stall;
  a.sidx = sidx;
  if (trim)
    return swk::launch_score<32, 4, false, false, false, true, true, false, false, 8, true, true>(
        a, W, 0, st, grid);
  return swk::launch_score<32, 4, false, false, false, true, true, false, false, 8, true>(
      a, W, 0, st, grid);
}

extern "C" hipError_t swk_launch_stream(int R, int gotoh, int f16, int pair, const uint8_t* res,
                                        size_t n, uint32_t ulen, const SwkStreamChunk* sc,
                                        const uint32_t* hflag, uint32_t* dflag, uint32_t nsc,
                                        uint32_t* tctr, const uint32_t* qtab, uint32_t nv,
                                        uint32_t S, uint32_t O, uint32_t E, uint32_t PS,
                                        uint32_t pad, int W, int32_t* scores, uint32_t pS1,
                                        uint32_t pS2, hipStream_t st) {
  if (n == 0) return hipSuccess;
  if (!sc || !hflag || !dflag || !tctr || nsc == 0) return hipErrorInvalidValue;
  swk::ScoreArgs a{res,  nullptr, nullptr, n, qtab, nv, S, O, E, PS, pad, scores, nullptr, nullptr,
                   0u, 0u, (uint32_t)SWK_PACK_STREAM, nullptr, nullptr, 0u, nullptr, pS1, pS2,
                   swk::f16_pair(-(int)(O + E)), swk::f16_pair(-(int)E),
                   swk::f16_pair(-(int)O), nullptr, 0u, 0u, 0};
  a.ulen = ulen;
  a.sc = sc;
  a.hflag = hflag;
  a.dflag = dflag;
  a.tctr = tctr;
  a.nsc = nsc;
  if (pair) {
    if (R == 32 && f16 && !gotoh)
      return swk::launch_score<32, 4, false, false, false, true, true, false, true>(a, W, 0, st);
    if (R == 32 && f16 && gotoh)
      return swk::launch_score<32, 4, false, false, true, true, true, false, true>(a, W, 0, st);
    if (R == 16 && f16 && gotoh)
      return swk::launch_score<16, 4, false, false, true, true, true, false, true>(a, W, 0, st);
    return hipErrorInvalidValue;
  }
#define SWK_ST_CASE(RR, GT, FH)                                                                  \
  if (R == RR && gotoh == GT && f16 == FH)                                                       \
    return swk::launch_score<RR, 4, false, false, (GT != 0), (FH != 0), false, false, true>(     \
        a, W, 0, st);
  SWK_ST_CASE(32, 0, 1) SWK_ST_CASE(32, 0, 0) SWK_ST_CASE(16, 0, 1) SWK_ST_CASE(16, 0, 0)
  SWK_ST_CASE(16, 1, 1) SWK_ST_CASE(16, 1, 0) SWK_ST_CASE(32, 1, 1) SWK_ST_CASE(32, 1, 0)
#undef SWK_ST_CASE
  return hipErrorInvalidValue;
}
```

smith-waterman-fpga-module_amd/csrc/swbank_launch.hip:

```cpp
#include "swbank_bank.h"

static bool one_len_bin(uint32_t min_len, uint32_t max_len) {
  if (min_len > max_len) return false;
  uint32_t shift = 0;
  while ((max_len >> shift) >= 2048u) ++shift;
  return ((max_len - min_len) >> shift) == 0;
}

void u16_gotoh_rows(const sw_bank* b, bool f16, int& R, int& W) {
  if (f16 || !b->gotoh() || b->prof || R != 32 || b->segs.size() != 1 || b->query.size() > 256)
    return;
  R = 16;
  W = std::max(1, (int)((b->query.size() + 15) / 16));
}

bool wave_preferred(const sw_bank* b, size_t n, uint32_t max_len, bool use_f16) {
  const size_t nseg = b->segs.size();
  const size_t ntiles = (n + SWB_TILE - 1) / SWB_TILE;
  const bool gotoh = b->cfg.gap_model == SW_GAP_GOTOH;
  const double tiles = (double)ntiles, W = b->segs[0].W;
  const double cu_frac = std::min(1.0, tiles / 256.0);
  const double wps = std::min(4.0, std::max(1.0, std::ceil(tiles / 256.0)) * W / 4.0);
  const bool pair_tab = use_f16 && b->pair_bytes != 0 && env_int("SWBANK_PAIR", 1) != 0;
  const double tile_base = use_f16 ? (gotoh ? (b->prof ? 7100 : pair_tab ? 8500 : 7500)
                                            : (b->prof ? 8000 : 9000))
                                   : (gotoh ? (b->prof ? 5600 : 5800) : (b->prof ? 6500 : 7400));
  const double tile_est = tile_base * cu_frac * std::min(1.0, 0.45 + 0.15 * wps) *
                          (nseg > 1 ? 0.85 : 1.0);
  double wave_est = 0;
  if (b->wK > 0) {
    const double rowfill = (double)b->query.size() / (64.0 * b->wK * b->wsegs);
    const double colfill = max_len / (max_len + 63.0);
    const double wave_base = use_f16 ? (gotoh ? (b->prof ? 6800 : 7800) : (b->prof ? 7700 : 8600))
                                     : (gotoh ? (b->prof ? 5200 : 6100) : (b->prof ? 6600 : 7600));
    wave_est = wave_base * rowfill * colfill *
               (b->wsegs > 1 ? 0.9 : 1.0);
  }
  const char* kforce = std::getenv("SWBANK_KERNEL");
  bool use_wave = b->wK > 0 && wave_est > tile_est;
  if (kforce && std::strcmp(kforce, "tile") == 0) use_wave = false;
  if (kforce && std::strcmp(kforce, "wave") == 0 && b->wK > 0) use_wave = true;
  return use_wave;
}

static uint32_t poll_limit(uint32_t dflt) {
  const int v = env_int("SWBANK_POLL_LIMIT", 0);
  return v > 0 ? (uint32_t)v : dflt;
}

static int ragged_trim() { return env_int("SWBANK_TRIM", 1) != 0 ? 1 : 0; }

sw_status launch(sw_bank* b, const uint8_t* d_res, const uint64_t* d_offs,
                 const uint32_t* d_lens, size_t n, uint32_t max_len, int32_t* d_scores,
                 hipStream_t st, uint32_t packed, const uint32_t* perm, const uint32_t* perm_n,
                 bool dsort, bool wait_prev, uint32_t* sort_out, uint32_t* sort_scr, uint32_t ulen,
                 uint32_t ustride, uint32_t min_len) {
  const uint64_t bound = std::min<uint64_t>(b->query.size(), max_len) *
                             (uint64_t)std::max(0, b->smax) + (uint64_t)std::max(0, b->smax);
  const bool need32 = bound > 65535u || env_int("SWBANK_I32", 0) != 0;
  if (need32 && ustride) return fail(b, SW_ERR_ARG, "uniform batch past the 16-bit bound");
  if (need32) {
    if (n > 0xFFFFFFFFull)
      return fail(b, SW_ERR_RANGE, "batches past the 16-bit score bound hold < 2^32 targets");
    const sw_status ps = prepare_i32(b);
    if (ps != SW_OK) return ps;
  }
  sw_bank::Ev ev{};
  if (b->timing) {
    HIPOK(b, hipEventCreate(&ev.a));
    HIPOK(b, hipEventCreate(&ev.c));
    HIPOK(b, hipEventRecord(ev.a, st));
    ev.b = ev.a;
  }
  HIPOK(b, hipStreamWaitEvent(st, b->ev_ready, 0));
  if (wait_prev) HIPOK(b, hipStreamWaitEvent(st, b->ev_used, 0));
  const size_t nseg = b->segs.size();
  const bool rec = packed == SWK_PACK_RECORDS;
  const uint32_t ecols = (max_len + 7) / 8 * 8;
  const size_t ntiles = (n + SWB_TILE - 1) / SWB_TILE;
  const bool gotoh = b->cfg.gap_model == SW_GAP_GOTOH;
  const uint64_t top = std::min<uint64_t>(b->query.size(), max_len) * (uint64_t)std::max(0, b->smax) +
                       (uint64_t)std::max(0, b->smax);
  const bool f16_ok = b->f16 && b->f16_neg >= -2048 && env_int("SWBANK_F16", 1) != 0;
  const bool exact16 = f16_ok && top <= 2048u;
  const bool opt16 = f16_ok && !exact16 && n <= 0xFFFFFFFFull;
  const bool use_f16 = exact16 || opt16;
  bool use_wave = wave_preferred(b, n, max_len, use_f16);
  if (packed == SWK_PACK_MIXED) use_wave = false;
  if (use_f16 && b->prof && (size_t)(b->alpha + 1) * b->wPS16 > 65536) use_wave = false;
  const char* arith = opt16 ? "f16+u16-rescore" : use_f16 ? "f16" : "u16";
  const bool use_pair = use_f16 && b->pair_bytes != 0 && env_int("SWBANK_PAIR", 1) != 0;
  bool wave_fb = false;
  if (use_wave) {
    const bool half = use_f16 && b->prof && !b->col0 && b->wK == 8 && b->wsegs == 1 &&
                      env_int("SWBANK_WAVE_HALF", 1) != 0;
    snprintf(b->last_kernel, sizeof(b->last_kernel), "wave %s%s K=%d segs=%d%s", arith,
             b->prof ? "-profile" : "", b->wK, b->wsegs, half ? " pairs/wave=2" : "");
    size_t wspan = n;
    if (b->wsegs > 1) {
      const size_t budget = (size_t)std::max(1, env_int("SWBANK_EDGE_MB", 2048)) << 20;
      wspan = std::min(n, std::max<size_t>(1, budget / ((size_t)ecols * sizeof(uint2))) * 2);
      const size_t words = std::max<size_t>(1, (wspan + 1) / 2 * ecols);
      HIPOK(b, b->edge[0].reserve(words));
      HIPOK(b, b->edge[1].reserve(words));
    }
    wave_fb = opt16 && b->wsegs == 1;
    SwkWaveSplit sp{};
    const size_t pairs = (n + 1) / 2;
    const int sforce = env_int("SWBANK_WAVE_SPLIT", -1);
    bool wbal = false;
    if (half && b->wsegs == 1 && n == wspan && !b->no_handoff && (ustride || min_len == max_len) &&
        sforce < 0 && pairs <= 0xFFFFFFFFull && env_int("SWBANK_WAVE_BAL", 1) != 0) {
      const size_t U = (pairs + 1) / 2, B = (max_len + 31 + 31) / 32;
      const int wforce = env_int("SWBANK_WAVE_W", 0);
      int W = wforce == 4 ? 4 : 8;
      unsigned grid = swk_wave_half_grid(gotoh ? 1 : 0, (b->pad + 1) * b->wPS16, W);
      bool ok = W == 8 && swk_wbal_admissible(U, B, 8, grid) &&
                (wforce == 8 || U >= (size_t)8 * grid);
      if (!ok) {
        W = 4;
        grid = swk_wave_half_grid(gotoh ? 1 : 0, (b->pad + 1) * b->wPS16, W);
        const size_t G4 = (size_t)4 * grid;
        ok = swk_wbal_admissible(U, B, 4, grid) && U >= G4 && U % G4;
      }
      const size_t G = (size_t)W * grid;
      uint32_t* fw = ok ? fault_word(b) : nullptr;
      if (ok && fw) {
        const size_t sw = (G + 1) * 36 * 64;
        HIPOK(b, b->wbal_state.reserve(sw));
        if (b->wbal_flag.cap < G + 1) {
          HIPOK(b, b->wbal_flag.reserve(G + 1));
          HIPOK(b, hipMemsetAsync(b->wbal_flag.p, 0, b->wbal_flag.cap * 4, st));
        }
        sp.wbal_blocks = (uint32_t)B;
        sp.wbal_grid = grid;
        sp.wbal_waves = (unsigned)W;
        sp.wbal_gen = ++b->wbal_gen;
        sp.wbal_flag = b->wbal_flag.p;
        sp.wbal_state = b->wbal_state.p;
        sp.fault = fw + (b->host_call ? SWK_FAULT_WORDS : 0);
        sp.poll_limit = poll_limit(1u << 23);
        sp.stall = (unsigned)std::max(0, env_int("SWBANK_STALL", 0));
        wbal = true;
        const size_t L = strlen(b->last_kernel);
        snprintf(b->last_kernel + L, sizeof(b->last_kernel) - L, " balanced grid=%ux%d", grid, W);
      }
    }
    if (!wbal && b->sK[0] && b->wsegs == 1 && n == wspan && pairs <= 0xFFFFFFFFull) {
      const size_t simds = 4 * (size_t)std::max(b->cus, 1);
      const size_t units = half ? 2 * simds : simds;
      size_t T = 0;
      if (sforce >= 0) T = std::min(pairs, (size_t)sforce);
      else if (pairs >= units && pairs % units <= units / 2) T = pairs % units;
      const int pforce = env_int("SWBANK_WAVE_SPLIT_P", 0);
      const bool seg8 = half && b->sK[2] == 1 && T && !b->no_handoff &&
                        (pforce == 8 || (!pforce && 8 * T <= simds));
      const int i = pforce == 2 ? 0 : pforce == 4 ? 1 : (4 * T <= simds ? 1 : 0);
      uint32_t* fw = seg8 ? fault_word(b) : nullptr;
      if (seg8 && !fw) return fail(b, SW_ERR_NOMEM, "fault word allocation failed");
      if (seg8) {
        HIPOK(b, b->sring.reserve(std::max<size_t>(1, T * 7 * (size_t)ecols)));
        const size_t pw = T * 8 * 3;
        HIPOK(b, b->tprog.reserve(pw));
        HIPOK(b, hipMemsetAsync(b->tprog.p, 0, pw * 4, st));
        sp.pairs = (unsigned)T;
        sp.P = 8;
        sp.qtab = b->stab16[2].p;
        sp.words = (unsigned)b->sseg_words16[2];
        sp.PS = b->sPS16[2];
        sp.ring = b->sring.p;
        sp.cols = ecols;
        sp.prog = b->tprog.p;
        sp.fault = fw + (b->host_call ? SWK_FAULT_WORDS : 0);
        sp.poll_limit = poll_limit(1u << 24);
        sp.stall = (unsigned)std::max(0, env_int("SWBANK_STALL", 0));
        const size_t L = strlen(b->last_kernel);
        snprintf(b->last_kernel + L, sizeof(b->last_kernel) - L, " tail=%zu/8", T);
      } else if (T && b->sK[i]) {
        const unsigned P = 2u << i;
        HIPOK(b, b->sring.reserve((T + 4 / P - 1) / (4 / P) * (4 / P) * (P - 1) * 256));
        sp.pairs = (unsigned)T;
        sp.P = P;
        sp.qtab = use_f16 ? b->stab16[i].p : b->stab[i].p;
        sp.words = (unsigned)(use_f16 ? b->sseg_words16[i] : b->sseg_words[i]);
        sp.PS = use_f16 && b->prof ? b->sPS16[i] : b->sPS[i];
        sp.fb_qtab = b->stab[i].p;
        sp.fb_words = (unsigned)b->sseg_words[i];
        sp.fb_PS = b->sPS[i];
        sp.ring = b->sring.p;
        const size_t L = strlen(b->last_kernel);
        snprintf(b->last_kernel + L, sizeof(b->last_kernel) - L, " split=%zu/%u", T, P);
      }
    }
    for (size_t p0 = 0; p0 < n; p0 += wspan) {
      const size_t np = std::min(wspan, n - p0);
      for (int sg = 0; sg < b->wsegs; ++sg) {
        const void* ein = sg > 0 ? b->edge[(sg - 1) & 1].p : nullptr;
        void* eout = sg + 1 < b->wsegs ? b->edge[sg & 1].p : nullptr;
        HIPOK(b, swk_launch_wave(
                     b->wK, b->col0, b->prof, gotoh ? 1 : 0, use_f16 ? 1 : 0, ein, eout, ecols,
                     sg > 0 ? 1 : 0, rec ? d_res + p0 * SWB_RECORD : d_res,
                     rec ? d_offs : d_offs + p0, rec ? d_lens : d_lens + p0, np,
                     use_f16 ? b->wtab16.p + sg * b->wseg_words16 : b->wtab.p + sg * b->wseg_words,
                     use_f16 ? b->nv16 : b->nv, b->S, b->O, b->E,
                     use_f16 && b->prof ? b->wPS16 : b->wPS, b->pad, d_scores + p0,
                     (int)packed, wave_fb ? b->wtab.p : nullptr, b->nv, b->wPS,
                     2048 - std::max(0, b->smax), &sp, ulen, ustride, half ? 1 : 0, st));
      }
    }
  } else {
    int R0 = b->R, W0 = b->segs[0].W;
    u16_gotoh_rows(b, use_f16, R0, W0);
    snprintf(b->last_kernel, sizeof(b->last_kernel), "tile %s%s R=%d W=%d segs=%zu", arith,
             b->prof ? "-profile" : use_pair ? " pair" : "", R0, W0, nseg);
  }
  const uint32_t* ident = nullptr;
  unsigned rbal_grid = 0;
  if (dsort && !sort_out && !b->no_handoff && !use_wave && !perm && use_f16 && use_pair && !gotoh && nseg == 1 &&
      wait_prev && (packed == SWK_PACK_BYTES || packed == SWK_PACK_NIBBLE) && min_len < max_len &&
      max_len < 2048 && !opt16 &&
      b->R == 32 && b->segs[0].W <= 4 && n <= 0xFFFFFFFFull && env_int("SWBANK_DSORT", 1) != 0 &&
      env_int("SWBANK_BAL", 1) != 0 && env_int("SWBANK_BAL_RAGGED", 1) != 0 &&
      !one_len_bin(min_len, max_len)) {
    const unsigned grid = swk_bal_slots(b->segs[0].W, b->pair_bytes, ragged_trim());
    const size_t kmin = std::max<uint32_t>(1u, (min_len + 7) / 8), kmax = (max_len + 7) / 8;
    if (grid && ntiles * kmin >= 2 * (size_t)grid * kmax && ntiles * kmax < (1ull << 31))
      rbal_grid = grid;
  }
  if (dsort && !use_wave && !perm && packed != SWK_PACK_RECORDS && ntiles > 1 &&
      n <= 0xFFFFFFFFull && !one_len_bin(min_len, max_len) && env_int("SWBANK_DSORT", 1) != 0) {
    uint32_t* order = sort_out;
    if (!order) {
      HIPOK(b, b->dperm.reserve(n + 2));
      order = b->dperm.p;
    }
    uint32_t* scr = sort_scr;
    if (!scr) {
      const size_t sw = swk_sort_scratch_bytes() / 4;
      if (b->dsort.cap < sw) {
        HIPOK(b, b->dsort.reserve(sw));
        HIPOK(b, hipMemsetAsync(b->dsort.p, 0, sw * 4, st));
      }
      scr = b->dsort.p;
    }
    if (rbal_grid) {
      HIPOK(b, b->bal_plan.reserve((size_t)(rbal_grid + 1) * 4));
      b->bal_key[0] = 0;
    }
    HIPOK(b, swk_sort_lens(d_lens, n, max_len, order, order + n, order + n + 1, scr, st,
                           rbal_grid ? b->bal_plan.p : nullptr, rbal_grid));
    ++b->ctr.device_sorts;
    if (!sort_out) {
      const size_t L = strlen(b->last_kernel);
      snprintf(b->last_kernel + L, sizeof(b->last_kernel) - L, " dsort");
    }
    perm = order;
    perm_n = order + n;
    ident = order + n + 1;
  }
  size_t span = n;
  if (nseg > 1) {
    const size_t budget = (size_t)std::max(1, env_int("SWBANK_EDGE_MB", 2048)) << 20;
    const size_t per_tile = (size_t)ecols * 64 * sizeof(uint2);
    span = std::max<size_t>(1, budget / std::max<size_t>(per_tile, 1)) * SWB_TILE;
    span = std::min(span, n);
    if (!use_wave || opt16) {
      const size_t words = std::max<size_t>(1, (span + SWB_TILE - 1) / SWB_TILE * ecols * 64);
      HIPOK(b, b->edge[0].reserve(words));
      HIPOK(b, b->edge[1].reserve(words));
    }
  }
  for (int pass = use_wave ? 1 : 0; pass < (opt16 && !wave_fb ? 2 : 1); ++pass) {
    const bool f16 = use_f16 && pass == 0;
    if (pass == 1) {
      HIPOK(b, b->fb_idx.reserve(n));
      HIPOK(b, b->fb_cnt.reserve(1));
      HIPOK(b, swk_flag_high(d_scores, n, 2048 - std::max(0, b->smax), b->fb_idx.p, b->fb_cnt.p,
                             st));
    }
    for (size_t p0 = 0; p0 < n; p0 += span) {
      const size_t np = std::min(span, n - p0);
      const uint8_t* res = d_res;
      const uint64_t* offs = d_offs;
      const uint32_t* lens = d_lens;
      int32_t* scores = d_scores;
      const uint32_t* idx = nullptr;
      const uint32_t* nidx = nullptr;
      if (pass == 0 && perm) {
        idx = perm + p0;
        nidx = perm_n;
      } else if (pass == 0 && rec) {
        res = d_res + p0 * SWB_RECORD;
        scores = d_scores + p0;
      } else if (pass == 0) {
        offs = d_offs + p0;
        lens = d_lens + p0;
        scores = d_scores + p0;
      } else {
        idx = b->fb_idx.p + p0;
        nidx = b->fb_cnt.p;
      }
      const bool rbal = pass == 0 && rbal_grid && perm && idx == perm && span == n;
      if (rbal || (pass == 0 && !b->no_handoff && f16 && use_pair && !gotoh && nseg == 1 && !idx && wait_prev &&
                   (packed == SWK_PACK_BYTES || packed == SWK_PACK_NIBBLE) && min_len == max_len &&
                   max_len > 0 && span == n &&
                   ntiles * ((max_len + 7) / 8) < (1ull << 31) && !opt16 && b->R == 32 &&
                   b->segs[0].W <= 4 && env_int("SWBANK_BAL", 1) != 0)) {
        const int Wl = b->segs[0].W;
        const unsigned grid = rbal ? rbal_grid : swk_bal_slots(Wl, b->pair_bytes, 0);
        uint32_t* fw = fault_word(b);
        if (!fw) return fail(b, SW_ERR_NOMEM, "fault word allocation failed");
        if (grid && (rbal || ntiles >= 2 * (size_t)grid)) {
          const size_t sw = (size_t)(grid + 1) * Wl * (2 * 32 + 2) * 64;
          HIPOK(b, b->bal_state.reserve(sw));
          if (b->bal_flag.cap < (size_t)(grid + 1) * Wl) {
            HIPOK(b, b->bal_flag.reserve((size_t)(grid + 1) * Wl));
            HIPOK(b, hipMemsetAsync(b->bal_flag.p, 0, b->bal_flag.cap * 4, st));
          }
          if (!rbal) {
            const size_t K = (max_len + 7) / 8;
            if (b->bal_key[0] != ntiles || b->bal_key[1] != K || b->bal_key[2] != grid) {
              HIPOK(b, b->bal_plan.reserve((size_t)(grid + 1) * 4));
              HIPOK(b, swk_bal_plan_uniform(b->bal_plan.p, (uint32_t)ntiles, (uint32_t)K, grid,
                                            st));
              b->bal_key[0] = ntiles;
              b->bal_key[1] = K;
              b->bal_key[2] = grid;
            }
          }
          const int gmode = rbal && ragged_trim() && packed == SWK_PACK_BYTES
                                ? env_int("SWBANK_RAGGED_GATHER", 0) : 0;
          const bool gat = gmode != 0;
          const bool gnib = gat && gmode == 2 && b->alpha <= 16;
          SwkDeal dl{};
          if (gat) {
            const size_t stride = ((gnib ? ((size_t)max_len + 7) / 8 * 4 : (size_t)max_len) + 15) &
                                  ~(size_t)15;
            HIPOK(b, b->gres.reserve(n * stride + 16));
            HIPOK(b, b->goffs.reserve(n));
            HIPOK(b, b->glens.reserve(n));
            dl.D = 1;
            dl.stride = (unsigned)stride;
            dl.codes[0] = b->gres.p;
            dl.offs[0] = reinterpret_cast<unsigned long long*>(b->goffs.p);
            dl.lens[0] = b->glens.p;
            dl.cnt[0] = n;
            dl.nib = gnib ? 1u : 0u;
            HIPOK(b, swk_deal_gather(res, offs, lens, idx, ident, n, &dl, st));
          }
          HIPOK(b, swk_launch_pair_bal(gat ? b->gres.p : res, gat ? b->goffs.p : offs,
                                       gat ? b->glens.p : lens, np, b->qpair.p, b->nv16, b->S, b->O,
                                       b->E, b->pair_bytes, b->pad, Wl,
                                       scores, b->pS1, b->pS2, ulen,
                                       ustride, b->bal_flag.p, b->bal_state.p, ++b->bal_gen, grid,
                                       gat ? nullptr : idx, gat ? nullptr : nidx,
                                       ident, b->bal_plan.p,
                                       fw + (b->host_call ? SWK_FAULT_WORDS : 0), poll_limit(1u << 23),
                                       (uint32_t)std::max(0, env_int("SWBANK_STALL", 0)),
                                       rbal && ragged_trim(),
                                       gnib ? (uint32_t)SWK_PACK_NIBBLE
                                            : gat ? (uint32_t)SWK_PACK_BYTES : packed,
                                       gat ? idx : nullptr, st));
          ++b->ctr.balanced_calls;
          const size_t L = strlen(b->last_kernel);
          snprintf(b->last_kernel + L, sizeof(b->last_kernel) - L, " balanced grid=%u%s", grid,
                   gnib ? " gather4" : gat ? " gather" : "");
          continue;
        }
      }
      for (size_t s = 0; s < nseg; ++s) {
        const void* ein = s > 0 ? b->edge[(s - 1) & 1].p : nullptr;
        void* eout = s + 1 < nseg ? b->edge[s & 1].p : nullptr;
        const bool pair = f16 && use_pair;
        int R = b->R, Wl = b->segs[s].W;
        u16_gotoh_rows(b, f16, R, Wl);
        HIPOK(b, swk_launch_score(R, b->RB, b->col0, b->prof, gotoh ? 1 : 0, f16 ? 1 : 0, res,
                                  offs, lens, np,
                                  pair ? b->qpair.p + s * (b->pair_bytes / 4)
                                  : f16 ? b->qtab16.p + b->segs[s].off16
                                        : b->qtab.p + b->segs[s].off,
                                  f16 ? b->nv16 : b->nv, b->S, b->O, b->E,
                                  pair ? b->pair_bytes : f16 && b->prof ? b->PS16 : b->PS,
                                  b->pad, Wl, scores, ein, eout, ecols, s > 0 ? 1 : 0,
                                  (int)packed, idx, nidx, (uint32_t)p0,
                                  pass == 0 ? ident : nullptr, pair ? 1 : 0, b->pS1, b->pS2,
                                  ulen, ustride, 1u, 0u, 0, st));
      }
    }
  }
  if (need32) {
    const uint32_t scols = std::max(max_len, 1u);
    const size_t budget = (size_t)std::max(1, env_int("SWBANK_EDGE_MB", 2048)) << 20;
    const size_t waves = swk_i32_waves(n, scols, budget);
    HIPOK(b, b->fb_idx.reserve(n));
    HIPOK(b, b->fb_cnt.reserve(1));
    HIPOK(b, b->i32scr.reserve(waves * 2 * scols));
    const int32_t thresh = bound > 65535u ? 65535 - std::max(0, b->smax) : -1;
    HIPOK(b, swk_flag_high(d_scores, n, thresh, b->fb_idx.p, b->fb_cnt.p, st));
    HIPOK(b, swk_launch_i32(gotoh ? 1 : 0, d_res, d_offs, d_lens, n, (int)packed, b->fb_idx.p,
                            b->fb_cnt.p, 0, b->i32prof.p, b->i32_strips,
                            (uint32_t)b->query.size(), b->pad, b->O, b->E, d_scores, b->i32scr.p,
                            scols, waves, st));
    const size_t L = strlen(b->last_kernel);
    snprintf(b->last_kernel + L, sizeof(b->last_kernel) - L, " +i32-rescore");
  }
  HIPOK(b, hipEventRecord(b->ev_used, st));
  if (b->timing) {
    HIPOK(b, hipEventRecord(ev.c, st));
    b->events.push_back(ev);
  }
  return SW_OK;
}

sw_status track_best_device(sw_bank* b, const int32_t* d_scores, const uint64_t* d_ids, size_t n,
                            hipStream_t st) {
  if (n > 0xFFFFFFFFull) return SW_OK;
  HIPOK(b, b->best_key.reserve(1));
  HIPOK(b, b->best_dev.reserve(3));
  HIPOK(b, swk_best_hit(d_scores, d_ids, n, b->best_key.p, b->best_dev.p, b->best_dev.p + 2, st));
  if (!b->best_ev) HIPOK(b, hipEventCreateWithFlags(&b->best_ev, hipEventDisableTiming));
  HIPOK(b, hipEventRecord(b->best_ev, st));
  b->best_kind = 2;
  return SW_OK;
}

sw_status launch_set(sw_bank* b, const uint8_t* d_res, const uint64_t* d_offs,
                     const uint32_t* d_lens, size_t n, uint32_t min_len, uint32_t max_len,
                     int32_t* d_scores, hipStream_t st, size_t sstride) {
  const size_t nq = b->qset.size();
  const uint64_t smax = (uint64_t)std::max(0, b->smax);
  const uint64_t top = std::min<uint64_t>(b->query.size(), max_len) * smax + smax;
  const bool f16_ok = b->f16 && b->f16_neg >= -2048 && env_int("SWBANK_F16", 1) != 0;
  const bool use_f16 = f16_ok && top <= 2048u;
  const bool exact = use_f16 || top <= 65535u;
  const size_t ntiles = (n + SWB_TILE - 1) / SWB_TILE;
  const char* kforce = std::getenv("SWBANK_KERNEL");
  const bool mq = env_int("SWBANK_MQ", 1) != 0 && !b->prof && !b->col0 && exact &&
                  env_int("SWBANK_I32", 0) == 0 && (b->R == 16 || b->R == 32) && b->RB == 4 &&
                  n <= 0xFFFFFFFFull &&
                  !(kforce && std::strcmp(kforce, "wave") == 0) && ntiles * nq <= 0x7FFFFFFFull;
  if (!mq) {
    const std::vector<uint8_t> longest = b->query;
    sw_status rs = SW_OK;
    for (size_t i = 0; i < nq && rs == SW_OK; ++i) {
      b->query = b->qset[i];
      b->dirty = true;
      rs = prepare(b);
      if (rs == SW_OK)
        rs = launch(b, d_res, d_offs, d_lens, n, max_len, d_scores + i * sstride, st, SWK_PACK_BYTES,
                    nullptr, nullptr, true, true, nullptr, nullptr, 0, 0, min_len);
    }
    b->query = longest;
    b->dirty = true;
    const size_t L = strlen(b->last_kernel);
    snprintf(b->last_kernel + L, sizeof(b->last_kernel) - L, " x%zu queries", nq);
    return rs;
  }
  sw_status rs = prepare_multi(b);
  if (rs != SW_OK) return rs;
  const bool gotoh = b->gotoh();
  const int prow = std::max(b->mq_pair_rows, 32);
  const size_t slots = (prow > 256 ? 1 : prow > 128 ? 2 : 4) * (size_t)std::max(b->cus, 1);
  const bool mpair = b->mq_pair_segs > 0 && use_f16 && nq <= slots &&
                     8 * (slots - slots / nq * nq) <= slots;
  const size_t nseg = mpair ? (size_t)b->mq_pair_segs : b->segs.size();
  snprintf(b->last_kernel, sizeof(b->last_kernel), "tile %s%s R=%d W=%d segs=%zu queries=%zu",
           use_f16 ? "f16" : "u16", mpair ? " pair" : "", b->R,
           mpair ? std::min(prow / 32, (int)(b->query.size() + 31) / 32) : b->segs[0].W, nseg,
           nq);
// ... 148 lines not shown
```

Measured before the change: 12770.

## Add skewed-offset f16 pair kernel variant for linear-gap Smith-Waterman

Adds a SKEW variant of the balanced and plain f16 pair score kernel for linear gaps. Substitution scores are pre-offset by twice the gap-extend penalty and a per-row floor table is kept in constant memory, so the inner recurrence uses fewer operations per cell (the per-cell gap subtraction is folded into the table and a running best offset). The path is enabled by default when range checks pass (scores fit in f16, single segment, exact16). It adds new table uploads, extra kernel template instantiations and a larger argument block, and relies on the f16 range bounds holding for correctness.

Result: faster. 13730, median of 6 (+7.5%).

```diff
diff --git a/smith-waterman-fpga-module_amd/csrc/swbank_bank.h b/smith-waterman-fpga-module_amd/csrc/swbank_bank.h
--- a/smith-waterman-fpga-module_amd/csrc/swbank_bank.h
+++ b/smith-waterman-fpga-module_amd/csrc/swbank_bank.h
@@ -53,8 +53,9 @@
                                        const uint32_t* nidx, uint32_t idx_base,
                                        const uint32_t* ident, int pair, uint32_t pS1,
                                        uint32_t pS2, uint32_t ulen, uint32_t ustride, uint32_t nq,
-                                       uint32_t qwords, size_t sstride, hipStream_t st);
-extern "C" unsigned swk_bal_slots(int W, uint32_t PS, int trim);
+                                       uint32_t qwords, size_t sstride, hipStream_t st,
+                                       const uint32_t* skew_tab = nullptr);
+extern "C" unsigned swk_bal_slots(int W, uint32_t PS, int trim, int skew = 0);
 extern "C" unsigned swk_wave_half_grid(int gotoh, uint32_t prof_bytes, int W);
 extern "C" hipError_t swk_bal_plan_uniform(void* plan, uint32_t ntiles, uint32_t K, uint32_t G,
                                            hipStream_t st);
@@ -68,7 +69,8 @@
                                           const uint32_t* nidx, const uint32_t* ident,
                                           const void* plan, uint32_t* fault, uint32_t poll_limit,
                                           uint32_t stall, int trim, uint32_t packed,
-                                          const uint32_t* sidx, hipStream_t st);
+                                          const uint32_t* sidx, hipStream_t st,
+                                          const uint32_t* skew_tab = nullptr);
 extern "C" hipError_t swk_best_hit(const int32_t* scores, const uint64_t* ids, size_t n,
                                    unsigned long long* key, uint64_t* out, uint64_t* out_index,
                                    hipStream_t st);
@@ -363,6 +365,9 @@
   DevBuf<uint32_t> qtab16;
   DevBuf<uint32_t> qpair;
   uint32_t pair_bytes = 0, pS1 = 0, pS2 = 0;
+  DevBuf<uint32_t> qpair_skew, skew_ctab;
+  uint32_t skew_entries = 0;
+  int32_t skew_neg = 0;
   DevBuf<uint32_t> fb_idx, fb_cnt;
   bool i32_ready = false;
   uint32_t i32_strips = 0;
diff --git a/smith-waterman-fpga-module_amd/csrc/swbank_bank.hip b/smith-waterman-fpga-module_amd/csrc/swbank_bank.hip
--- a/smith-waterman-fpga-module_amd/csrc/swbank_bank.hip
+++ b/smith-waterman-fpga-module_amd/csrc/swbank_bank.hip
@@ -169,6 +169,8 @@
   b->mqtab16.release();
   b->mqpair.release();
   b->qpair.release();
+  b->qpair_skew.release();
+  b->skew_ctab.release();
   b->stage.release();
   if (b->ev_ready) (void)hipEventDestroy(b->ev_ready);
   if (b->ev_used) (void)hipEventDestroy(b->ev_used);
@@ -491,13 +493,16 @@
 }
 
 static std::vector<uint32_t> pair_table(const uint8_t* q, int qlen, int r0, uint32_t NR,
-                                        const int8_t* m, int A, uint32_t pS1, uint32_t pS2) {
+                                        const int8_t* m, int A, uint32_t pS1, uint32_t pS2,
+                                        int add = 0, int pad = -2048) {
   const uint32_t bytes = 16 + 4 * pS1 + 4 * pS2 + 4 * NR;
-  std::vector<uint32_t> t(bytes / 4, 0xBC00BC00u);
+  const uint32_t padw = (uint32_t)f16_score_bits(pad + add) * 0x10001u;
+  std::vector<uint32_t> t(bytes / 4, padw);
   auto word = [&](int r, int x, int y) -> uint32_t {
-    if (r0 + r >= qlen) return 0xBC00BC00u;
+    if (r0 + r >= qlen) return padw;
     const int c = q[r0 + r];
-    return (uint32_t)f16_score_bits(m[c * A + x]) | (uint32_t)f16_score_bits(m[c * A + y]) << 16;
+    return (uint32_t)f16_score_bits(m[c * A + x] + add) |
+           (uint32_t)f16_score_bits(m[c * A + y] + add) << 16;
   };
   for (int x = 0; x < A; ++x)
     for (int y = 0; y < A; ++y) {
@@ -647,6 +652,17 @@
       pair_words = (uint32_t)t.size();
       tpair.insert(tpair.end(), t.begin(), t.end());
     }
+  }
+  std::vector<uint32_t> tskew, tfloor;
+  int skew_neg = 0;
+  if (!tpair.empty() && !gotoh && 2 * e <= 2048) {
+    const int spad = -std::min(2048 - 2 * e, S * std::max(qlen, 1));
+    tskew = pair_table(b->query.data(), qlen, 0, (uint32_t)segs[0].W * R, m, A, pS1, pS2, 2 * e,
+                       spad);
+    tfloor.resize(2048 + 192);
+    for (size_t k = 0; k < tfloor.size(); ++k)
+      tfloor[k] = (uint32_t)f16_score_bits(std::min(2048, e * ((int)k - 3))) * 0x10001u;
+    skew_neg = -3 * e + std::min(smin, spad) + 2 * e - o;
   }
   const auto wave_tables = [&](int wrows, int nsegs, std::vector<uint32_t>& wt,
                                std::vector<uint32_t>& wt16) {
@@ -716,7 +732,8 @@
   HIPOK(b, hipEventSynchronize(b->ev_ready));
   const size_t nbytes =
       (wt16.size() + wt.size() + st16[0].size() + st[0].size() + st16[1].size() +
-       st[1].size() + st16[2].size() + st[2].size() + tab.size() + tab16.size() + tpair.size()) *
+       st[1].size() + st16[2].size() + st[2].size() + tab.size() + tab16.size() + tpair.size() +
+       tskew.size() + tfloor.size()) *
       4;
   HIPOK(b, b->stage.reserve(nbytes));
   HIPOK(b, hipStreamWaitEvent(b->stream, b->ev_used, 0));
@@ -749,6 +766,12 @@
   HIPOK(b, upload(b->qtab, tab));
   if (f16) HIPOK(b, upload(b->qtab16, tab16));
   if (!tpair.empty()) HIPOK(b, upload(b->qpair, tpair));
+  if (!tskew.empty()) {
+    HIPOK(b, upload(b->qpair_skew, tskew));
+    HIPOK(b, upload(b->skew_ctab, tfloor));
+  }
+  b->skew_entries = tskew.empty() ? 0u : (uint32_t)tfloor.size();
+  b->skew_neg = skew_neg;
   b->pair_bytes = pair_words * 4;
   b->pS1 = pS1;
   b->pS2 = pS2;
diff --git a/smith-waterman-fpga-module_amd/csrc/swbank_f16_rows.inc b/smith-waterman-fpga-module_amd/csrc/swbank_f16_rows.inc
--- a/smith-waterman-fpga-module_amd/csrc/swbank_f16_rows.inc
+++ b/smith-waterman-fpga-module_amd/csrc/swbank_f16_rows.inc
@@ -1348,6 +1348,132 @@
   "v_pk_maximum3_f16 %[F], 0, %[HN], %[FN]\n\t" \
   "v_pk_maximum3_f16 %[best], %[best], %[h6], %[h7]\n\t" \
   ""
+#define SWK_F16SKEW_F \
+  "v_pk_add_f16 %[Da], %[dg], %[pw]\n\t" \
+  "v_pk_add_f16 %[Db], %[h0], %[p0]\n\t" \
+  "v_pk_add_f16 %[AO], %[Da], %[no]\n\t" \
+  "v_pk_add_f16 %[best], %[best], %[e2f]\n\t" \
+  "v_pk_maximum3_f16 %[t0], %[AO], %[up], %[t0]\n\t" \
+  "v_pk_add_f16 %[AO], %[Db], %[no]\n\t" \
+  "v_pk_maximum3_f16 %[h0], %[t0], %[Da], %[c0]\n\t" \
+  "v_pk_add_f16 %[Da], %[h1], %[p1]\n\t" \
+  "v_pk_maximum3_f16 %[best], %[best], %[h0], %[h1]\n\t" \
+  "v_pk_maximum3_f16 %[t1], %[AO], %[t0], %[t1]\n\t" \
+  "v_pk_add_f16 %[AO], %[Da], %[no]\n\t" \
+  "v_pk_maximum3_f16 %[h1], %[t1], %[Db], %[c1]\n\t" \
+  "v_pk_add_f16 %[Db], %[h2], %[p2]\n\t" \
+  "v_pk_maximum3_f16 %[t2], %[AO], %[t1], %[t2]\n\t" \
+  "v_pk_add_f16 %[AO], %[Db], %[no]\n\t" \
+  "v_pk_add_f16 %[best], %[best], %[e2]\n\t" \
+  "v_pk_maximum3_f16 %[h2], %[t2], %[Da], %[c2]\n\t" \
+  "v_pk_add_f16 %[Da], %[h3], %[p3]\n\t" \
+  "v_pk_maximum3_f16 %[best], %[best], %[h2], %[h3]\n\t" \
+  "v_pk_maximum3_f16 %[t3], %[AO], %[t2], %[t3]\n\t" \
+  "v_pk_add_f16 %[AO], %[Da], %[no]\n\t" \
+  "v_pk_maximum3_f16 %[h3], %[t3], %[Db], %[c3]\n\t" \
+  "v_pk_add_f16 %[Db], %[h4], %[p4]\n\t" \
+  "v_pk_maximum3_f16 %[t4], %[AO], %[t3], %[t4]\n\t" \
+  "v_pk_add_f16 %[AO], %[Db], %[no]\n\t" \
+  "v_pk_add_f16 %[best], %[best], %[e2]\n\t" \
+  "v_pk_maximum3_f16 %[h4], %[t4], %[Da], %[c4]\n\t" \
+  "v_pk_add_f16 %[Da], %[h5], %[p5]\n\t" \
+  "v_pk_maximum3_f16 %[best], %[best], %[h4], %[h5]\n\t" \
+  "v_pk_maximum3_f16 %[t5], %[AO], %[t4], %[t5]\n\t" \
+  "v_pk_add_f16 %[AO], %[Da], %[no]\n\t" \
+  "v_pk_maximum3_f16 %[h5], %[t5], %[Db], %[c5]\n\t" \
+  "v_pk_add_f16 %[Db], %[h6], %[p6]\n\t" \
+  "v_pk_maximum3_f16 %[t6], %[AO], %[t5], %[t6]\n\t" \
+  "v_pk_add_f16 %[AO], %[Db], %[no]\n\t" \
+  "v_pk_add_f16 %[best], %[best], %[e2]\n\t" \
+  "v_pk_maximum3_f16 %[h6], %[t6], %[Da], %[c6]\n\t" \
+  "v_pk_add_f16 %[Da], %[h7], %[p7]\n\t" \
+  "v_pk_maximum3_f16 %[best], %[best], %[h6], %[h7]\n\t" \
+  "v_pk_maximum3_f16 %[t7], %[AO], %[t6], %[t7]\n\t" \
+  "v_pk_add_f16 %[AO], %[Da], %[no]\n\t" \
+  "v_pk_maximum3_f16 %[h7], %[t7], %[Db], %[c7]\n\t" \
+  ""
+#define SWK_F16SKEW_M \
+  "v_pk_add_f16 %[Db], %[h0], %[p0]\n\t" \
+  "v_pk_maximum3_f16 %[t0], %[AO], %[up], %[t0]\n\t" \
+  "v_pk_add_f16 %[AO], %[Db], %[no]\n\t" \
+  "v_pk_add_f16 %[best], %[best], %[e2]\n\t" \
+  "v_pk_maximum3_f16 %[h0], %[t0], %[Da], %[c0]\n\t" \
+  "v_pk_add_f16 %[Da], %[h1], %[p1]\n\t" \
+  "v_pk_maximum3_f16 %[best], %[best], %[h0], %[h1]\n\t" \
+  "v_pk_maximum3_f16 %[t1], %[AO], %[t0], %[t1]\n\t" \
+  "v_pk_add_f16 %[AO], %[Da], %[no]\n\t" \
+  "v_pk_maximum3_f16 %[h1], %[t1], %[Db], %[c1]\n\t" \
+  "v_pk_add_f16 %[Db], %[h2], %[p2]\n\t" \
+  "v_pk_maximum3_f16 %[t2], %[AO], %[t1], %[t2]\n\t" \
+  "v_pk_add_f16 %[AO], %[Db], %[no]\n\t" \
+  "v_pk_add_f16 %[best], %[best], %[e2]\n\t" \
+  "v_pk_maximum3_f16 %[h2], %[t2], %[Da], %[c2]\n\t" \
+  "v_pk_add_f16 %[Da], %[h3], %[p3]\n\t" \
+  "v_pk_maximum3_f16 %[best], %[best], %[h2], %[h3]\n\t" \
+  "v_pk_maximum3_f16 %[t3], %[AO], %[t2], %[t3]\n\t" \
+  "v_pk_add_f16 %[AO], %[Da], %[no]\n\t" \
+  "v_pk_maximum3_f16 %[h3], %[t3], %[Db], %[c3]\n\t" \
+  "v_pk_add_f16 %[Db], %[h4], %[p4]\n\t" \
+  "v_pk_maximum3_f16 %[t4], %[AO], %[t3], %[t4]\n\t" \
+  "v_pk_add_f16 %[AO], %[Db], %[no]\n\t" \
+  "v_pk_add_f16 %[best], %[best], %[e2]\n\t" \
+  "v_pk_maximum3_f16 %[h4], %[t4], %[Da], %[c4]\n\t" \
+  "v_pk_add_f16 %[Da], %[h5], %[p5]\n\t" \
+  "v_pk_maximum3_f16 %[best], %[best], %[h4], %[h5]\n\t" \
+  "v_pk_maximum3_f16 %[t5], %[AO], %[t4], %[t5]\n\t" \
+  "v_pk_add_f16 %[AO], %[Da], %[no]\n\t" \
+  "v_pk_maximum3_f16 %[h5], %[t5], %[Db], %[c5]\n\t" \
+  "v_pk_add_f16 %[Db], %[h6], %[p6]\n\t" \
+  "v_pk_maximum3_f16 %[t6], %[AO], %[t5], %[t6]\n\t" \
+  "v_pk_add_f16 %[AO], %[Db], %[no]\n\t" \
+  "v_pk_add_f16 %[best], %[best], %[e2]\n\t" \
+  "v_pk_maximum3_f16 %[h6], %[t6], %[Da], %[c6]\n\t" \
+  "v_pk_add_f16 %[Da], %[h7], %[p7]\n\t" \
+  "v_pk_maximum3_f16 %[best], %[best], %[h6], %[h7]\n\t" \
+  "v_pk_maximum3_f16 %[t7], %[AO], %[t6], %[t7]\n\t" \
+  "v_pk_add_f16 %[AO], %[Da], %[no]\n\t" \
+  "v_pk_maximum3_f16 %[h7], %[t7], %[Db], %[c7]\n\t" \
+  ""
+#define SWK_F16SKEW_L \
+  "v_pk_add_f16 %[Db], %[h0], %[p0]\n\t" \
+  "v_pk_maximum3_f16 %[t0], %[AO], %[up], %[t0]\n\t" \
+  "v_pk_add_f16 %[AO], %[Db], %[no]\n\t" \
+  "v_pk_add_f16 %[best], %[best], %[e2]\n\t" \
+  "v_pk_maximum3_f16 %[h0], %[t0], %[Da], %[c0]\n\t" \
+  "v_pk_add_f16 %[Da], %[h1], %[p1]\n\t" \
+  "v_pk_maximum3_f16 %[best], %[best], %[h0], %[h1]\n\t" \
+  "v_pk_maximum3_f16 %[t1], %[AO], %[t0], %[t1]\n\t" \
+  "v_pk_add_f16 %[AO], %[Da], %[no]\n\t" \
+  "v_pk_maximum3_f16 %[h1], %[t1], %[Db], %[c1]\n\t" \
+  "v_pk_add_f16 %[Db], %[h2], %[p2]\n\t" \
+  "v_pk_maximum3_f16 %[t2], %[AO], %[t1], %[t2]\n\t" \
+  "v_pk_add_f16 %[AO], %[Db], %[no]\n\t" \
+  "v_pk_add_f16 %[best], %[best], %[e2]\n\t" \
+  "v_pk_maximum3_f16 %[h2], %[t2], %[Da], %[c2]\n\t" \
+  "v_pk_add_f16 %[Da], %[h3], %[p3]\n\t" \
+  "v_pk_maximum3_f16 %[best], %[best], %[h2], %[h3]\n\t" \
+  "v_pk_maximum3_f16 %[t3], %[AO], %[t2], %[t3]\n\t" \
+  "v_pk_add_f16 %[AO], %[Da], %[no]\n\t" \
+  "v_pk_maximum3_f16 %[h3], %[t3], %[Db], %[c3]\n\t" \
+  "v_pk_add_f16 %[Db], %[h4], %[p4]\n\t" \
+  "v_pk_maximum3_f16 %[t4], %[AO], %[t3], %[t4]\n\t" \
+  "v_pk_add_f16 %[AO], %[Db], %[no]\n\t" \
+  "v_pk_add_f16 %[best], %[best], %[e2]\n\t" \
+  "v_pk_maximum3_f16 %[h4], %[t4], %[Da], %[c4]\n\t" \
+  "v_pk_add_f16 %[Da], %[h5], %[p5]\n\t" \
+  "v_pk_maximum3_f16 %[best], %[best], %[h4], %[h5]\n\t" \
+  "v_pk_maximum3_f16 %[t5], %[AO], %[t4], %[t5]\n\t" \
+  "v_pk_add_f16 %[AO], %[Da], %[no]\n\t" \
+  "v_pk_maximum3_f16 %[h5], %[t5], %[Db], %[c5]\n\t" \
+  "v_pk_add_f16 %[Db], %[h6], %[p6]\n\t" \
+  "v_pk_maximum3_f16 %[t6], %[AO], %[t5], %[t6]\n\t" \
+  "v_pk_add_f16 %[AO], %[Db], %[no]\n\t" \
+  "v_pk_add_f16 %[best], %[best], %[e2]\n\t" \
+  "v_pk_maximum3_f16 %[h6], %[t6], %[Da], %[c6]\n\t" \
+  "v_pk_maximum3_f16 %[t7], %[AO], %[t6], %[t7]\n\t" \
+  "v_pk_maximum3_f16 %[best], %[best], %[h6], %[h7]\n\t" \
+  "v_pk_maximum3_f16 %[h7], %[t7], %[Db], %[c7]\n\t" \
+  ""
 #define SWK_F16M_F_Z0_L0 \
   "v_pk_fma_f16 %[Db], %[fa0], %[fb0], %[h0] op_sel:[0,1,0] op_sel_hi:[1,0,1] clamp\n\t" \
   "v_pk_add_f16 %[DN], %[Da], %[no]\n\t" \
diff --git a/smith-waterman-fpga-module_amd/csrc/swbank_kcommon.h b/smith-waterman-fpga-module_amd/csrc/swbank_kcommon.h
--- a/smith-waterman-fpga-module_amd/csrc/swbank_kcommon.h
+++ b/smith-waterman-fpga-module_amd/csrc/swbank_kcommon.h
@@ -604,8 +604,10 @@
   uint32_t poll_limit, stall;
   uint32_t wbal_blocks, wbal_grid;
   const uint32_t* sidx;
+  const uint32_t* ctab;
+  uint32_t f16_e2, f16_e2f;
 };
-static_assert(sizeof(ScoreArgs) == 376, "ScoreArgs layout (kernel argument block) changed");
+static_assert(sizeof(ScoreArgs) == 392, "ScoreArgs layout (kernel argument block) changed");
 
 __device__ __forceinline__ void report_fault(uint32_t* fault, uint32_t bit) {
   if (fault) __hip_atomic_store(fault + __builtin_ctz(bit), bit, __ATOMIC_RELAXED,
diff --git a/smith-waterman-fpga-module_amd/csrc/swbank_ktile.hip b/smith-waterman-fpga-module_amd/csrc/swbank_ktile.hip
--- a/smith-waterman-fpga-module_amd/csrc/swbank_ktile.hip
+++ b/smith-waterman-fpga-module_amd/csrc/swbank_ktile.hip
@@ -6,10 +6,13 @@
 #define SWK_TRIM_BREAK 1
 #endif
 template <int R, int RB, bool COL0, bool PROF, bool GOTOH, bool F16, bool PAIR = false,
-          bool MQ = false, bool STREAM = false, int C = 8, bool BAL = false, bool TRIM = false>
+          bool MQ = false, bool STREAM = false, int C = 8, bool BAL = false, bool TRIM = false,
+          bool SKEW = false>
 __global__ void __launch_bounds__(R >= 64 ? 512 : 1024) score_kernel(const ScoreArgs a) {
   static_assert(!BAL || (!MQ && !STREAM && !COL0), "balanced ranges: one query, resident batch");
   static_assert(!TRIM || (BAL && PAIR), "trimmed last chunks: the balanced pair kernel");
+  static_assert(!SKEW || (PAIR && F16 && !GOTOH && !MQ && !STREAM && R == 32 && C == 8),
+                "SKEW: the merged f16 pair rows, one query, resident batch");
   static_assert(!MQ || !PROF, "several queries: row-LUT or pair-table variants");
   static_assert(!STREAM || (!MQ && !PROF), "streamed batches: single-query LUT / pair variants");
   static_assert(C == 8 || (C == 4 && PAIR && !STREAM), "4-column chunks: pair tables only");
@@ -43,7 +46,14 @@
   uint32_t packed = a.packed;
   int* sq = reinterpret_cast<int*>(prof);
   int bs = 0, bo = 0, be = 0, bf = 0;
-  if constexpr (BAL) {
+  if constexpr (BAL && SKEW) {
+    typedef __attribute__((address_space(4))) const uint32_t plan_u32;
+    plan_u32* const pp = reinterpret_cast<plan_u32*>(reinterpret_cast<uintptr_t>(a.bal_plan)) +
+                         (size_t)blockIdx.x * 4;
+    bs = (int)pp[0], bo = (int)pp[1];
+    be = (int)pp[4], bf = (int)pp[5];
+    total = (int)(pp[6] - pp[2]);
+  } else if constexpr (BAL) {
     const uint4 p0 = a.bal_plan[blockIdx.x], p1 = a.bal_plan[blockIdx.x + 1];
     bs = (int)__builtin_amdgcn_readfirstlane(p0.x), bo = (int)__builtin_amdgcn_readfirstlane(p0.y);
     be = (int)__builtin_amdgcn_readfirstlane(p1.x), bf = (int)__builtin_amdgcn_readfirstlane(p1.y);
@@ -62,9 +72,11 @@
     } else {
       t = nunits, c0 = 0, c1 = 1;
     }
-    t = __builtin_amdgcn_readfirstlane(t);
-    c0 = __builtin_amdgcn_readfirstlane(c0);
-    c1 = __builtin_amdgcn_readfirstlane(c1);
+    if constexpr (!SKEW) {
+      t = __builtin_amdgcn_readfirstlane(t);
+      c0 = __builtin_amdgcn_readfirstlane(c0);
+      c1 = __builtin_amdgcn_readfirstlane(c1);
+    }
   };
   if constexpr (BAL) {
   } else if constexpr (STREAM) {
@@ -157,6 +169,26 @@
   for (int i = threadIdx.x; i < W * SWB_TILE; i += blockDim.x) bestsh[i] = 0;
   const f16x2 NOE2 = as_f16x2(as_u16x2(a.f16_noe)), NE2 = as_f16x2(as_u16x2(a.f16_ne)),
               NO2 = as_f16x2(as_u16x2(a.f16_no));
+  typedef __attribute__((address_space(4))) const uint32_t cst_u32;
+  cst_u32* const ct = reinterpret_cast<cst_u32*>(reinterpret_cast<uintptr_t>(a.ctab));
+  constexpr uint32_t SKEW_NEG = 0xBC00BC00u;
+  uint32_t skew_c0 = 0;
+  if constexpr (SKEW) skew_c0 = ct[wave * R + 1];
+  const auto skew_reset = [&](u16x2 (&H)[R], u16x2 (&X)[R], u16x2& bst, u16x2& pup) {
+    uint32_t c0 = skew_c0;
+    asm volatile("" : "+v"(c0));
+    f16x2 h = as_f16x2(__builtin_bit_cast(u16x2, c0));
+    const f16x2 ne = as_f16x2(as_u16x2(a.f16_ne));
+    pup = as_u16x2(h + ne);
+#pragma unroll
+    for (int r = 0; r < R; ++r) {
+      H[r] = as_u16x2(h);
+      X[r] = __builtin_bit_cast(u16x2, SKEW_NEG);
+      h = h - ne;
+    }
+    bst = H[R - 2];
+  };
+  (void)ct; (void)skew_reset;
   if (wave == 0) {
     if (lane < C)
       ring[lane * RS + 64] = F16 ? make_uint2(0u, GOTOH ? 0u : as_u32(as_u16x2(NOE2)))
@@ -197,6 +229,7 @@
   }
   u16x2 best = {0, 0};
   u16x2 prevUpH = H0;
+  if constexpr (SKEW) skew_reset(Hl, Xl, best, prevUpH);
   uint2 rlo, rhi;
   load_raw<C, !MQ>(cur, vc0, vc0 < nfull, a.pad, packed, rlo, rhi);
   if (STREAM && threadIdx.x == 0) sq[W] = total;
@@ -372,6 +405,18 @@
       uint2* rout = wave < W - 1 ? ring + ((size_t)(wave * 2 + slot) * C) * RS + lane
                     : W > 1      ? rin
                                  : ring + lane;
+      const int cu = __builtin_amdgcn_readfirstlane(c);
+      uint32_t cs[SKEW ? R + C : 1];
+      if constexpr (SKEW) {
+        cst_u32* const sl = ct + (wave * R + cu * C + 1);
+#pragma unroll
+        for (int s = 0; s < R + C; ++s) cs[s] = sl[s];
+        if (wave == 0 && lane == 0) {
+#pragma unroll
+          for (int jj = 0; jj < C; ++jj) ring[jj * RS + 64] = make_uint2(cs[jj], SKEW_NEG);
+        }
+      }
+      (void)cu; (void)cs;
       uint2 rv = rin[0];
       ProfLookup16<PROF && F16 ? R : 2> lkq;
       (void)lkq;
@@ -442,6 +487,59 @@
           } else {
             column_merged<R, RB, false>(lk, diag, upX, Hl, Xl, best, S2, O2, E2);
           }
+        } else if constexpr (PAIR && SKEW) {
+          const uint32_t nwl = jj + 1 < C ? (jj + 1 < 4 ? clo.x : clo.y) : rlo.x;
+          const uint32_t nwh = jj + 1 < C ? (jj + 1 < 4 ? chi.x : chi.y) : rhi.x;
+          const int nsh = jj + 1 < C ? 8 * ((jj + 1) & 3) : 0;
+          uint32_t Da, Db, AO;
+          const uint32_t no = as_u32(as_u16x2(NO2)), e2 = a.f16_e2, e2f = a.f16_e2f;
+          u16x2 bst = best;
+#define SWK_SKEW_OUT(B, DA)                                                                   \
+  [h0] "+v"(Hl[B]), [h1] "+v"(Hl[B + 1]), [h2] "+v"(Hl[B + 2]), [h3] "+v"(Hl[B + 3]),          \
+      [h4] "+v"(Hl[B + 4]), [h5] "+v"(Hl[B + 5]), [h6] "+v"(Hl[B + 6]), [h7] "+v"(Hl[B + 7]),  \
+      [t0] "+v"(Xl[B]), [t1] "+v"(Xl[B + 1]), [t2] "+v"(Xl[B + 2]), [t3] "+v"(Xl[B + 3]),      \
+      [t4] "+v"(Xl[B + 4]), [t5] "+v"(Xl[B + 5]), [t6] "+v"(Xl[B + 6]), [t7] "+v"(Xl[B + 7]),  \
+      [Db] "=&v"(Db), [best] "+v"(bst), [Da] DA(Da), [AO] DA(AO)
+#define SWK_SKEW_IN(B, P0, P1)                                                                \
+  [p0] "v"(P0.x), [p1] "v"(P0.y), [p2] "v"(P0.z), [p3] "v"(P0.w), [p4] "v"(P1.x),             \
+      [p5] "v"(P1.y), [p6] "v"(P1.z), [p7] "v"(P1.w), [no] "s"(no), [e2] "s"(e2),             \
+      [c0] "s"(cs[B + jj + 1]), [c1] "s"(cs[B + jj + 2]), [c2] "s"(cs[B + jj + 3]),           \
+      [c3] "s"(cs[B + jj + 4]), [c4] "s"(cs[B + jj + 5]), [c5] "s"(cs[B + jj + 6]),           \
+      [c6] "s"(cs[B + jj + 7]), [c7] "s"(cs[B + jj + 8])
+#define SWK_SKEW_BLOCK(KIND, B, P0, P1)                                                       \
+  if constexpr (KIND == 0)                                                                    \
+    asm volatile(SWK_F16SKEW_F : SWK_SKEW_OUT(B, "=&v")                                       \
+                 : SWK_SKEW_IN(B, P0, P1), [e2f] "s"(e2f), [up] "v"(upX), [dg] "v"(diag),     \
+                   [pw] "v"(pw));                                                             \
+  else if constexpr (KIND == 1)                                                               \
+    asm volatile(SWK_F16SKEW_M : SWK_SKEW_OUT(B, "+v") : SWK_SKEW_IN(B, P0, P1),              \
+                 [up] "v"(Xl[B - 1]));                                                        \
+  else                                                                                        \
+    asm volatile(SWK_F16SKEW_L : SWK_SKEW_OUT(B, "+v") : SWK_SKEW_IN(B, P0, P1),              \
+                 [up] "v"(Xl[B - 1]));
+          uint4 pB0 = ld4(acur + 48), pB1 = ld4(acur + 64);
+          __builtin_amdgcn_sched_barrier(0);
+          SWK_SKEW_BLOCK(0, 0, pA0, pA1)
+          pA0 = ld4(acur + 80);
+          pA1 = ld4(acur + 96);
+          __builtin_amdgcn_sched_barrier(0);
+          SWK_SKEW_BLOCK(1, 8, pB0, pB1)
+          pB0 = ld4(acur + 112);
+          pB1 = ld4(acur + 128);
+          __builtin_amdgcn_sched_barrier(0);
+          SWK_SKEW_BLOCK(1, 16, pA0, pA1)
+          acur = pair_addr(nwl, nwh, nsh);
+          pA0 = ld4(acur + 16);
+          pA1 = ld4(acur + 32);
+          pw = ld1(acur + 12);
+          __builtin_amdgcn_sched_barrier(0);
+          SWK_SKEW_BLOCK(2, R - 8, pB0, pB1)
+#undef SWK_SKEW_BLOCK
+#undef SWK_SKEW_OUT
+#undef SWK_SKEW_IN
+          (void)Db; (void)AO;
+          best = bst;
+          upX = Xl[R - 1];
         } else if constexpr (PAIR) {
           const uint32_t nwl = jj + 1 < C ? (jj + 1 < 4 ? clo.x : clo.y) : rlo.x;
           const uint32_t nwh = jj + 1 < C ? (jj + 1 < 4 ? chi.x : chi.y) : rhi.x;
@@ -552,14 +650,30 @@
         if (BAL && k == 0 && bf > 0) {
           bal_store((int)blockIdx.x + 1);
         } else {
+        if constexpr (SKEW) {
+          f16x2 bb = as_f16x2(best);
+          const f16x2 e2 = as_f16x2(as_u16x2(a.f16_e2)), e2f = as_f16x2(as_u16x2(a.f16_e2f));
+#pragma unroll
+          for (int r = 1; r < R; r += 2) bb = fmax2(bb + (r == 1 ? e2f : e2), as_f16x2(Hl[r]));
+          const uint32_t cf =
+              ct[__builtin_amdgcn_readfirstlane(wave * R + R + 1 + cu * C + ncols - 1)];
+          best = as_u16x2(bb - as_f16x2(__builtin_bit_cast(u16x2, cf)));
+        }
         uint32_t* bs = bestsh + (k % W) * SWB_TILE;
-        atomicMax(&bs[lane], (uint32_t)best.x);
-        atomicMax(&bs[lane + 64], (uint32_t)best.y);
+        if constexpr (SKEW) {
+          uint32_t ol = (uint32_t)lane;
+          asm volatile("" : "+v"(ol));
+          bs += ol;
+        } else {
+          bs += lane;
+        }
+        atomicMax(&bs[0], (uint32_t)best.x);
+        atomicMax(&bs[64], (uint32_t)best.y);
         if (wave == W - 1) {
           const size_t tlo = (size_t)tile * SWB_TILE + lane, thi = tlo + 64;
-          int32_t blo = (int32_t)bs[lane], bhi = (int32_t)bs[lane + 64];
-          bs[lane] = 0;
-          bs[lane + 64] = 0;
+          int32_t blo = (int32_t)bs[0], bhi = (int32_t)bs[64];
+          bs[0] = 0;
+          bs[64] = 0;
           if constexpr (F16) {
             blo = f16_unscore((uint32_t)blo);
             bhi = f16_unscore((uint32_t)bhi);
@@ -590,6 +704,7 @@
         }
         best = (u16x2){0, 0};
         prevUpH = H0;
+        if constexpr (SKEW) skew_reset(Hl, Xl, best, prevUpH);
         tile = ntile;
         if constexpr (STREAM) {
           packed = packed_n;
@@ -663,13 +778,14 @@
 }
 
 template <int R, int RB, bool COL0, bool PROF, bool GOTOH, bool F16, bool PAIR = false,
-          bool MQ = false, bool STREAM = false, int C = 8, bool BAL = false, bool TRIM = false>
+          bool MQ = false, bool STREAM = false, int C = 8, bool BAL = false, bool TRIM = false,
+          bool SKEW = false>
 static hipError_t launch_score(const ScoreArgs& a, int W, uint32_t prof_bytes, hipStream_t st,
                                unsigned bal_grid = 0) {
   const size_t ntiles = (a.n + SWB_TILE - 1) / SWB_TILE * (MQ ? a.nq : 1);
   const size_t lds = (size_t)W * SWB_TILE * 4 + tile_ring_entries(W, C, a.edge_in != nullptr) * 8 +
                      (PROF ? prof_bytes : 0) + (PAIR ? a.PS : 0) + (STREAM ? 256 : 0);
-  auto fn = &score_kernel<R, RB, COL0, PROF, GOTOH, F16, PAIR, MQ, STREAM, C, BAL, TRIM>;
+  auto fn = &score_kernel<R, RB, COL0, PROF, GOTOH, F16, PAIR, MQ, STREAM, C, BAL, TRIM, SKEW>;
   static bool attr_set = false;
   if (!attr_set) {
     hipError_t e = hipFuncSetAttribute(reinterpret_cast<const void*>(fn),
@@ -692,6 +808,12 @@
   if (BAL && (grid == 0 || ntiles < 2 * (size_t)grid)) return hipErrorInvalidConfiguration;
   hipLaunchKernelGGL(fn, dim3(grid), dim3(64 * W), (unsigned)lds, st, a);
   return hipGetLastError();
+}
+
+static void skew_args(ScoreArgs& a, const uint32_t* tab, int R) {
+  a.ctab = tab;
+  a.f16_e2 = f16_pair(2 * (int)a.E);
+  a.f16_e2f = f16_pair((3 - R) * (int)a.E);
 }
 
 }
@@ -727,7 +849,7 @@
                                        const uint32_t* ident, int pair, uint32_t pS1,
                                        uint32_t pS2, uint32_t ulen, uint32_t ustride,
                                        uint32_t nq, uint32_t qwords, size_t sstride,
-                                       hipStream_t st) {
+                                       hipStream_t st, const uint32_t* skew_tab) {
   if (n == 0) return hipSuccess;
   swk::ScoreArgs a{res,  offs, lens, n,  qtab, nv, S,
                    O,    E,    PS,   pad, scores, static_cast<const uint2*>(edge_in),
@@ -758,6 +880,13 @@
     return hipErrorInvalidValue;
   }
   if (pair) {
+    if (skew_tab && (R != 32 || !f16 || prof || gotoh || col0 || edge_in || edge_out || W > 4))
+      return hipErrorInvalidValue;
+    if (skew_tab) {
+      swk::skew_args(a, skew_tab, 32);
+      return swk::launch_score<32, 4, false, false, false, true, true, false, false, 8, false,
+                               false, true>(a, W, 0, st);
+    }
     if (R == 32 && f16 && !prof && !gotoh && !col0)
       return swk::launch_score<32, 4, false, false, false, true, true>(a, W, 0, st);
 #define SWK_GPAIR(RR)                                                                         \
@@ -804,9 +933,15 @@
   return hipGetLastError();
 }
 
-extern "C" unsigned swk_bal_slots(int W, uint32_t PS, int trim) {
+extern "C" unsigned swk_bal_slots(int W, uint32_t PS, int trim, int skew) {
   const void* fn =
-      trim ? reinterpret_cast<const void*>(
+      skew ? (trim ? reinterpret_cast<const void*>(
+                         &swk::score_kernel<32, 4, false, false, false, true, true, false, false,
+                                            8, true, true, true>)
+                   : reinterpret_cast<const void*>(
+                         &swk::score_kernel<32, 4, false, false, false, true, true, false, false,
+                                            8, true, false, true>))
+      : trim ? reinterpret_cast<const void*>(
                  &swk::score_kernel<32, 4, false, false, false, true, true, false, false, 8, true,
                                     true>)
            : reinterpret_cast<const void*>(
@@ -831,7 +966,8 @@
                                           const uint32_t* nidx, const uint32_t* ident,
                                           const void* plan, uint32_t* fault, uint32_t poll_limit,
                                           uint32_t stall, int trim, uint32_t packed,
-                                          const uint32_t* sidx, hipStream_t st) {
+                                          const uint32_t* sidx, hipStream_t st,
+                                          const uint32_t* skew_tab) {
   if (n == 0) return hipSuccess;
   if (W > 4 || !flag || !state || !plan || !fault || poll_limit == 0 || (idx && !nidx) ||
       (packed != SWK_PACK_BYTES && packed != SWK_PACK_NIBBLE) || (sidx && (!trim || idx)))
@@ -852,6 +988,14 @@
   a.poll_limit = poll_limit;
   a.stall = stall;
   a.sidx = sidx;
+  if (skew_tab) {
+    swk::skew_args(a, skew_tab, 32);
+    if (trim)
+      return swk::launch_score<32, 4, false, false, false, true, true, false, false, 8, true, true,
+                               true>(a, W, 0, st, grid);
+    return swk::launch_score<32, 4, false, false, false, true, true, false, false, 8, true, false,
+                             true>(a, W, 0, st, grid);
+  }
   if (trim)
     return swk::launch_score<32, 4, false, false, false, true, true, false, false, 8, true, true>(
         a, W, 0, st, grid);
diff --git a/smith-waterman-fpga-module_amd/csrc/swbank_launch.hip b/smith-waterman-fpga-module_amd/csrc/swbank_launch.hip
--- a/smith-waterman-fpga-module_amd/csrc/swbank_launch.hip
+++ b/smith-waterman-fpga-module_amd/csrc/swbank_launch.hip
@@ -90,6 +90,13 @@
   if (use_f16 && b->prof && (size_t)(b->alpha + 1) * b->wPS16 > 65536) use_wave = false;
   const char* arith = opt16 ? "f16+u16-rescore" : use_f16 ? "f16" : "u16";
   const bool use_pair = use_f16 && b->pair_bytes != 0 && env_int("SWBANK_PAIR", 1) != 0;
+  const uint64_t skew_cols = ((uint64_t)max_len + 7) / 8 * 8;
+  const bool skew =
+      exact16 && use_pair && !gotoh && nseg == 1 && b->skew_entries != 0 && wait_prev &&
+      (packed == SWK_PACK_BYTES || packed == SWK_PACK_NIBBLE) &&
+      top + (uint64_t)b->E * ((uint64_t)b->segs[0].W * b->R + skew_cols) <= 2048u &&
+      b->skew_neg >= -2048 && skew_cols + 136 <= b->skew_entries &&
+      env_int("SWBANK_SKEW", 1) != 0;
   bool wave_fb = false;
   if (use_wave) {
     const bool half = use_f16 && b->prof && !b->col0 && b->wK == 8 && b->wsegs == 1 &&
@@ -211,8 +218,8 @@
   } else {
     int R0 = b->R, W0 = b->segs[0].W;
     u16_gotoh_rows(b, use_f16, R0, W0);
-    snprintf(b->last_kernel, sizeof(b->last_kernel), "tile %s%s R=%d W=%d segs=%zu", arith,
-             b->prof ? "-profile" : use_pair ? " pair" : "", R0, W0, nseg);
+    snprintf(b->last_kernel, sizeof(b->last_kernel), "tile %s%s R=%d W=%d segs=%zu%s", arith,
+             b->prof ? "-profile" : use_pair ? " pair" : "", R0, W0, nseg, skew ? " skew" : "");
   }
   const uint32_t* ident = nullptr;
   unsigned rbal_grid = 0;
@@ -222,7 +229,7 @@
       b->R == 32 && b->segs[0].W <= 4 && n <= 0xFFFFFFFFull && env_int("SWBANK_DSORT", 1) != 0 &&
       env_int("SWBANK_BAL", 1) != 0 && env_int("SWBANK_BAL_RAGGED", 1) != 0 &&
       !one_len_bin(min_len, max_len)) {
-    const unsigned grid = swk_bal_slots(b->segs[0].W, b->pair_bytes, ragged_trim());
+    const unsigned grid = swk_bal_slots(b->segs[0].W, b->pair_bytes, ragged_trim(), skew ? 1 : 0);
     const size_t kmin = std::max<uint32_t>(1u, (min_len + 7) / 8), kmax = (max_len + 7) / 8;
     if (grid && ntiles * kmin >= 2 * (size_t)grid * kmax && ntiles * kmax < (1ull << 31))
       rbal_grid = grid;
@@ -307,7 +314,8 @@
                    ntiles * ((max_len + 7) / 8) < (1ull << 31) && !opt16 && b->R == 32 &&
                    b->segs[0].W <= 4 && env_int("SWBANK_BAL", 1) != 0)) {
         const int Wl = b->segs[0].W;
-        const unsigned grid = rbal ? rbal_grid : swk_bal_slots(Wl, b->pair_bytes, 0);
+        const unsigned grid = rbal ? rbal_grid
+                                   : swk_bal_slots(Wl, b->pair_bytes, 0, skew ? 1 : 0);
         uint32_t* fw = fault_word(b);
         if (!fw) return fail(b, SW_ERR_NOMEM, "fault word allocation failed");
         if (grid && (rbal || ntiles >= 2 * (size_t)grid)) {
@@ -349,7 +357,8 @@
             HIPOK(b, swk_deal_gather(res, offs, lens, idx, ident, n, &dl, st));
           }
           HIPOK(b, swk_launch_pair_bal(gat ? b->gres.p : res, gat ? b->goffs.p : offs,
-                                       gat ? b->glens.p : lens, np, b->qpair.p, b->nv16, b->S, b->O,
+                                       gat ? b->glens.p : lens, np,
+                                       skew ? b->qpair_skew.p : b->qpair.p, b->nv16, b->S, b->O,
                                        b->E, b->pair_bytes, b->pad, Wl,
                                        scores, b->pS1, b->pS2, ulen,
                                        ustride, b->bal_flag.p, b->bal_state.p, ++b->bal_gen, grid,
@@ -360,7 +369,8 @@
                                        rbal && ragged_trim(),
                                        gnib ? (uint32_t)SWK_PACK_NIBBLE
                                             : gat ? (uint32_t)SWK_PACK_BYTES : packed,
-                                       gat ? idx : nullptr, st));
+                                       gat ? idx : nullptr, st,
+                                       skew ? b->skew_ctab.p : nullptr));
           ++b->ctr.balanced_calls;
           const size_t L = strlen(b->last_kernel);
           snprintf(b->last_kernel + L, sizeof(b->last_kernel) - L, " balanced grid=%u%s", grid,
@@ -376,7 +386,8 @@
         u16_gotoh_rows(b, f16, R, Wl);
         HIPOK(b, swk_launch_score(R, b->RB, b->col0, b->prof, gotoh ? 1 : 0, f16 ? 1 : 0, res,
                                   offs, lens, np,
-                                  pair ? b->qpair.p + s * (b->pair_bytes / 4)
+                                  pair && skew ? b->qpair_skew.p
+                                  : pair       ? b->qpair.p + s * (b->pair_bytes / 4)
                                   : f16 ? b->qtab16.p + b->segs[s].off16
                                         : b->qtab.p + b->segs[s].off,
                                   f16 ? b->nv16 : b->nv, b->S, b->O, b->E,
@@ -384,7 +395,8 @@
                                   b->pad, Wl, scores, ein, eout, ecols, s > 0 ? 1 : 0,
                                   (int)packed, idx, nidx, (uint32_t)p0,
                                   pass == 0 ? ident : nullptr, pair ? 1 : 0, b->pS1, b->pS2,
-                                  ulen, ustride, 1u, 0u, 0, st));
+                                  ulen, ustride, 1u, 0u, 0, st,
+                                  pair && skew ? b->skew_ctab.p : nullptr));
       }
     }
   }
```
